# DJjjjhao/FIRA-ICSE

Measured on NVIDIA H100. Metric: train_commits_per_sec, higher is better.
Workload: dtype bf16

## Files before the change

fira_icse_b200/csrc/common.cuh:

```cuda
#pragma once
#include <cuda_runtime.h>
#include <cuda_bf16.h>
#include <stdint.h>
#include <stdio.h>

#define FIRA_OK 0
#define FIRA_ERR_SHAPE 1
#define FIRA_ERR_ALIGN 2
#define FIRA_ERR_CUDA 3
#define FIRA_ERR_DTYPE 4
#define FIRA_ERR_ARG 5

#define FIRA_F32 0
#define FIRA_BF16 1

void fira_set_error(int code, const char* fmt, ...);

#define FIRA_CHECK_ARG(cond, code, ...)                      \
  do {                                                       \
    if (!(cond)) {                                           \
      fira_set_error((code), __VA_ARGS__);                   \
      return (code);                                         \
    }                                                        \
  } while (0)

#define FIRA_CHECK_LAUNCH(name)                                                   \
  do {                                                                            \
    cudaError_t e__ = cudaGetLastError();                                         \
    if (e__ != cudaSuccess) {                                                     \
      fira_set_error(FIRA_ERR_CUDA, "%s: %s", (name), cudaGetErrorString(e__));   \
      return FIRA_ERR_CUDA;                                                       \
    }                                                                             \
  } while (0)

extern "C" int fira_num_sms(void);

static inline bool fira_aligned16(const void* p) { return (reinterpret_cast<uintptr_t>(p) & 15u) == 0; }

int fira_pdl_on();

#ifdef __CUDACC__

__device__ __forceinline__ void pdl_wait() { asm volatile("griddepcontrol.wait;" ::: "memory"); }
__device__ __forceinline__ void pdl_trigger() { asm volatile("griddepcontrol.launch_dependents;" ::: "memory"); }

template <typename... KArgs, typename... Args>
inline cudaError_t launch_k(void (*kernel)(KArgs...), dim3 grid, dim3 block, size_t smem, cudaStream_t st, Args&&... args) {
  cudaLaunchConfig_t cfg = {};
  cfg.gridDim = grid;
  cfg.blockDim = block;
  cfg.dynamicSmemBytes = smem;
  cfg.stream = st;
  cudaLaunchAttribute attr[1];
  attr[0].id = cudaLaunchAttributeProgrammaticStreamSerialization;
  attr[0].val.programmaticStreamSerializationAllowed = 1;
  cfg.attrs = attr;
  cfg.numAttrs = fira_pdl_on() ? 1 : 0;
  return cudaLaunchKernelEx(&cfg, kernel, static_cast<KArgs>(args)...);
}

constexpr int kWarp = 32;
constexpr float kLnEps = 1e-5f;
constexpr float kMaskFill = -1e9f;

__device__ __forceinline__ float warp_sum(float v) {
#pragma unroll
  for (int o = 16; o > 0; o >>= 1) v += __shfl_xor_sync(0xffffffffu, v, o);
  return v;
}
__device__ __forceinline__ float warp_max(float v) {
#pragma unroll
  for (int o = 16; o > 0; o >>= 1) v = fmaxf(v, __shfl_xor_sync(0xffffffffu, v, o));
  return v;
}

template <typename T> struct Act;
template <> struct Act<float> {
  static __device__ __forceinline__ void load8(const float* p, float* v) {
    float4 a = *reinterpret_cast<const float4*>(p);
    float4 b = *reinterpret_cast<const float4*>(p + 4);
    v[0] = a.x; v[1] = a.y; v[2] = a.z; v[3] = a.w; v[4] = b.x; v[5] = b.y; v[6] = b.z; v[7] = b.w;
  }
  static __device__ __forceinline__ void store8(float* p, const float* v) {
    *reinterpret_cast<float4*>(p) = make_float4(v[0], v[1], v[2], v[3]);
    *reinterpret_cast<float4*>(p + 4) = make_float4(v[4], v[5], v[6], v[7]);
  }
  static __device__ __forceinline__ float ld(const float* p) { return *p; }
  static __device__ __forceinline__ void st(float* p, float v) { *p = v; }
};
template <> struct Act<__nv_bfloat16> {
  static __device__ __forceinline__ void load8(const __nv_bfloat16* p, float* v) {
    uint4 r = *reinterpret_cast<const uint4*>(p);
    const __nv_bfloat162* h = reinterpret_cast<const __nv_bfloat162*>(&r);
#pragma unroll
    for (int i = 0; i < 4; ++i) { float2 f = __bfloat1622float2(h[i]); v[2 * i] = f.x; v[2 * i + 1] = f.y; }
  }
  static __device__ __forceinline__ void store8(__nv_bfloat16* p, const float* v) {
    uint4 r;
    __nv_bfloat162* h = reinterpret_cast<__nv_bfloat162*>(&r);
#pragma unroll
    for (int i = 0; i < 4; ++i) h[i] = __floats2bfloat162_rn(v[2 * i], v[2 * i + 1]);
    *reinterpret_cast<uint4*>(p) = r;
  }
  static __device__ __forceinline__ float ld(const __nv_bfloat16* p) { return __bfloat162float(*p); }
  static __device__ __forceinline__ void st(__nv_bfloat16* p, float v) { *p = __float2bfloat16_rn(v); }
};

__device__ __forceinline__ uint4 philox4(uint32_t c0, uint32_t c1, uint32_t c2, uint32_t c3,
                                         uint32_t k0, uint32_t k1) {
  const uint32_t M0 = 0xD2511F53u, M1 = 0xCD9E8D57u, W0 = 0x9E3779B9u, W1 = 0xBB67AE85u;
#pragma unroll
  for (int r = 0; r < 7; ++r) {
    uint32_t hi0 = __umulhi(M0, c0), lo0 = M0 * c0;
    uint32_t hi1 = __umulhi(M1, c2), lo1 = M1 * c2;
    uint32_t n0 = hi1 ^ c1 ^ k0, n2 = hi0 ^ c3 ^ k1;
    c0 = n0; c1 = lo1; c2 = n2; c3 = lo0;
    k0 += W0; k1 += W1;
  }
  return make_uint4(c0, c1, c2, c3);
}
__device__ __forceinline__ uint32_t dropout_keep8(uint64_t seed, uint32_t stream, uint64_t idx8, float p_drop) {
  const uint4 r = philox4((uint32_t)idx8, (uint32_t)(idx8 >> 32), stream, 0u, (uint32_t)seed, (uint32_t)(seed >> 32));
  const uint32_t thr = (uint32_t)(p_drop * 65536.0f);
  uint32_t m = 0;
  m |= ((r.x & 0xffffu) >= thr) << 0; m |= ((r.x >> 16) >= thr) << 1;
  m |= ((r.y & 0xffffu) >= thr) << 2; m |= ((r.y >> 16) >= thr) << 3;
  m |= ((r.z & 0xffffu) >= thr) << 4; m |= ((r.z >> 16) >= thr) << 5;
  m |= ((r.w & 0xffffu) >= thr) << 6; m |= ((r.w >> 16) >= thr) << 7;
  return m;
}

#endif
```

fira_icse_b200/csrc/gemm_ln.cu:

```cuda
#include <cuda.h>
#include <cudaTypedefs.h>
#include "tc_common.cuh"
#include "fira_b200.h"

namespace {

using namespace tc;

constexpr int BM = 128, BN = 256, BK = 64, STAGES = 3;
constexpr int N_CONSUMER = 256;
constexpr int THREADS = N_CONSUMER + 32;
constexpr uint32_t A_BYTES = BM * BK * 2, B_BYTES = BN * BK * 2, STAGE_BYTES = A_BYTES + B_BYTES;
constexpr uint32_t RING_BYTES = STAGES * STAGE_BYTES;
constexpr uint32_t RES_BYTES = BM * BN * 2;
constexpr uint32_t SMEM_BYTES = RING_BYTES + RES_BYTES + 1024;
constexpr uint32_t BOX = 64 * 64 * 2;
constexpr uint32_t OFF_OUT = 8 * BOX;

struct LnParams {
  int M, K;
  long split;
  const float* bias; const float* rs; const float* rc; const float* gamma; const float* beta;
  float* mean; float* rstd;
  float p_drop; uint64_t seed; const uint64_t* seed_ctr; uint32_t stream_id;
  int has_b;
};

__global__ void __launch_bounds__(THREADS, 1)
gemm_ln_kernel(const __grid_constant__ CUtensorMap tmX, const __grid_constant__ CUtensorMap tmW,
               const __grid_constant__ CUtensorMap tmR, const __grid_constant__ CUtensorMap tmZ,
               const __grid_constant__ CUtensorMap tmOA, const __grid_constant__ CUtensorMap tmOB, LnParams p) {
  extern __shared__ unsigned char smem_dyn[];
  __shared__ __align__(8) unsigned long long full_bar[STAGES], empty_bar[STAGES], res_bar;
  __shared__ __align__(16) float s_bias[BN], s_rc[BN], s_gamma[BN], s_beta[BN];
  const uint32_t base = (smem_addr(smem_dyn) + 1023u) & ~1023u;
  unsigned char* sm = smem_dyn + (base - smem_addr(smem_dyn));
  const int warp = threadIdx.x >> 5, lane = threadIdx.x & 31;
  const int m0 = blockIdx.x * BM;
  const int nkb = (p.K + BK - 1) / BK;

  if (threadIdx.x == 0) {
    for (int s = 0; s < STAGES; ++s) { mbar_init(smem_addr(&full_bar[s]), 1); mbar_init(smem_addr(&empty_bar[s]), N_CONSUMER); }
    mbar_init(smem_addr(&res_bar), 1);
    mbar_init_fence();
    tma_prefetch_desc(&tmX); tma_prefetch_desc(&tmW); tma_prefetch_desc(&tmR); tma_prefetch_desc(&tmZ);
    tma_prefetch_desc(&tmOA);
    if (p.has_b) tma_prefetch_desc(&tmOB);
  }
  __syncthreads();
  pdl_wait(); pdl_trigger();

  if (warp == N_CONSUMER / 32) {
    if (lane == 0) {
      for (int i = 0; i < nkb; ++i) {
        const int s = i % STAGES;
        mbar_wait(smem_addr(&empty_bar[s]), ((i / STAGES) & 1) ^ 1);
        const uint32_t sa = base + s * STAGE_BYTES, sb = sa + A_BYTES, fb = smem_addr(&full_bar[s]);
        mbar_expect_tx(fb, STAGE_BYTES);
        const int kb = (i + (int)blockIdx.x) % nkb;
        tma_load_2d(sa, &tmX, kb * BK, m0, fb);
        tma_load_2d(sb, &tmW, kb * BK, 0, fb);
        if (i == 0) {
          const uint32_t rb = smem_addr(&res_bar);
          mbar_expect_tx(rb, RES_BYTES);
#pragma unroll
          for (int g = 0; g < 4; ++g) tma_load_2d(base + RING_BYTES + g * 16384, &tmR, g * 64, m0, rb);
        }
      }
    }
    return;
  }

  const int wg = warp >> 2;
  for (int c = threadIdx.x; c < BN; c += N_CONSUMER) {
    s_bias[c] = p.bias ? p.bias[c] : 0.f;
    s_rc[c] = p.rs ? p.rc[c] : 0.f;
    s_gamma[c] = p.gamma[c];
    s_beta[c] = p.beta[c];
  }
  float acc[BN / 2];
#pragma unroll
  for (int i = 0; i < BN / 2; ++i) acc[i] = 0.f;
  for (int i = 0; i < nkb; ++i) {
    const int s = i % STAGES;
    mbar_wait(smem_addr(&full_bar[s]), (i / STAGES) & 1);
    const uint32_t sa = base + s * STAGE_BYTES + wg * 8192, sb = base + s * STAGE_BYTES + A_BYTES;
    wgmma_fence();
#pragma unroll
    for (int k = 0; k < BK / 16; ++k) wgmma<BN, 0, 0>(acc, make_desc(sa + k * 32, 16, 1024), make_desc(sb + k * 32, 16, 1024));
    wgmma_commit();
    wgmma_wait<1>();
    if (i > 0) mbar_arrive(smem_addr(&empty_bar[(i - 1) % STAGES]));
  }
  wgmma_wait<0>();
  reg_fence<BN / 2>(acc);
  named_bar(1, N_CONSUMER);
  mbar_wait(smem_addr(&res_bar), 0);

  const int q4 = lane & 3;
  int tr[2], br[2], m[2];
  float rsm[2];
#pragma unroll
  for (int h = 0; h < 2; ++h) {
    tr[h] = wg * 64 + (warp & 3) * 16 + (lane >> 2) + 8 * h;
    br[h] = tr[h] - wg * 64;
    m[h] = m0 + tr[h];
    rsm[h] = (p.rs && m[h] < p.M) ? p.rs[m[h]] : 0.f;
  }
  uint64_t seed = p.seed;
  if (p.seed_ctr) seed += *p.seed_ctr;
  const float keep_scale = p.p_drop > 0.f ? 1.f / (1.f - p.p_drop) : 1.f;
  const unsigned char* res = sm + RING_BYTES;
  unsigned char* zst = sm + wg * 4 * BOX;
  unsigned char* ost = sm + OFF_OUT + wg * 4 * BOX;
  const int row0 = m0 + wg * 64;
  float sum[2] = {0.f, 0.f}, sq[2] = {0.f, 0.f};
#pragma unroll
  for (int j = 0; j < BN / 8; ++j) {
    const int c = 8 * j + 2 * q4, g = j >> 3, chunk = j & 7;
    const float2 bb = *reinterpret_cast<const float2*>(s_bias + c), kk = *reinterpret_cast<const float2*>(s_rc + c);
#pragma unroll
    for (int h = 0; h < 2; ++h) {
      float v0 = fmaf(rsm[h], kk.x, acc[4 * j + 2 * h] + bb.x), v1 = fmaf(rsm[h], kk.y, acc[4 * j + 2 * h + 1] + bb.y);
      const __nv_bfloat162 zb = __floats2bfloat162_rn(v0, v1);
      *reinterpret_cast<__nv_bfloat162*>(zst + g * BOX + br[h] * 128 + ((chunk ^ (br[h] & 7)) << 4) + q4 * 4) = zb;
      const float2 zf = __bfloat1622float2(zb);
      v0 = zf.x; v1 = zf.y;
      if (p.p_drop > 0.f) {
        const uint32_t mk = dropout_keep8(seed, p.stream_id, (uint64_t)m[h] * 32 + j, p.p_drop) >> (2 * q4);
        v0 = (mk & 1) ? v0 * keep_scale : 0.f;
        v1 = (mk & 2) ? v1 * keep_scale : 0.f;
      }
      const float2 rf = __bfloat1622float2(*reinterpret_cast<const __nv_bfloat162*>(
          res + g * 16384 + tr[h] * 128 + ((chunk ^ (tr[h] & 7)) << 4) + q4 * 4));
      v0 += rf.x; v1 += rf.y;
      acc[4 * j + 2 * h] = v0; acc[4 * j + 2 * h + 1] = v1;
      sum[h] += v0 + v1;
      sq[h] = fmaf(v0, v0, fmaf(v1, v1, sq[h]));
    }
  }
  fence_proxy_async();
  named_bar(2 + wg, 128);
  if ((threadIdx.x & 127) == 0 && row0 < p.M) {
#pragma unroll
    for (int g = 0; g < 4; ++g) tma_store_2d(&tmZ, smem_addr(zst + g * BOX), g * 64, row0);
    asm volatile("cp.async.bulk.commit_group;" ::: "memory");
  }
  float mean[2], rstd[2];
#pragma unroll
  for (int h = 0; h < 2; ++h) {
    sum[h] += __shfl_xor_sync(0xffffffffu, sum[h], 1);
    sum[h] += __shfl_xor_sync(0xffffffffu, sum[h], 2);
    sq[h] += __shfl_xor_sync(0xffffffffu, sq[h], 1);
    sq[h] += __shfl_xor_sync(0xffffffffu, sq[h], 2);
    mean[h] = sum[h] * (1.f / BN);
    const float var = fmaxf(sq[h] * (1.f / BN) - mean[h] * mean[h], 0.f);
    rstd[h] = rsqrtf(var + kLnEps);
    if (q4 == 0 && m[h] < p.M) { p.mean[m[h]] = mean[h]; p.rstd[m[h]] = rstd[h]; }
  }
#pragma unroll
  for (int j = 0; j < BN / 8; ++j) {
    const int c = 8 * j + 2 * q4, g = j >> 3, chunk = j & 7;
    const float2 gg = *reinterpret_cast<const float2*>(s_gamma + c), ee = *reinterpret_cast<const float2*>(s_beta + c);
#pragma unroll
    for (int h = 0; h < 2; ++h) {
      const float o0 = fmaf((acc[4 * j + 2 * h] - mean[h]) * rstd[h], gg.x, ee.x);
      const float o1 = fmaf((acc[4 * j + 2 * h + 1] - mean[h]) * rstd[h], gg.y, ee.y);
      *reinterpret_cast<__nv_bfloat162*>(ost + g * BOX + br[h] * 128 + ((chunk ^ (br[h] & 7)) << 4) + q4 * 4) =
          __floats2bfloat162_rn(o0, o1);
    }
  }
  fence_proxy_async();
  named_bar(2 + wg, 128);
  if ((threadIdx.x & 127) == 0) {
    if (row0 < p.M) {
#pragma unroll
      for (int g = 0; g < 4; ++g) {
        if (row0 < p.split) tma_store_2d(&tmOA, smem_addr(ost + g * BOX), g * 64, row0);
#pragma unroll
        for (int hh = 0; hh < 2; ++hh)
          if (p.has_b && row0 + 32 * hh < p.M && row0 + 32 * hh + 32 > p.split)
            tma_store_2d(&tmOB, smem_addr(ost + g * BOX + hh * 4096), g * 64, row0 + 32 * hh);
      }
    }
    tma_store_commit_wait_read();
  }
}

}

extern "C" int fira_gemm_ln_fwd(const void* x, long ldx, const void* w, const float* bias, const float* rs, const float* rc,
                                const void* resid, const float* gamma, const float* beta, void* z, void* outA, void* outB,
                                long split, float* mean, float* rstd, long rows, int K, float p_drop, uint64_t seed,
                                const uint64_t* seed_ctr, uint32_t stream_id, void* stream) {
  FIRA_CHECK_ARG(x && w && resid && gamma && beta && z && outA && mean && rstd, FIRA_ERR_ARG, "gemm_ln_fwd: null argument");
  FIRA_CHECK_ARG(rows > 0 && rows < (1L << 31) && K > 0 && K % 8 == 0, FIRA_ERR_SHAPE, "gemm_ln_fwd: rows %ld K %d", rows, K);
  FIRA_CHECK_ARG(ldx % 8 == 0, FIRA_ERR_ALIGN, "gemm_ln_fwd: ldx must be a multiple of 8");
  FIRA_CHECK_ARG(fira_aligned16(x) && fira_aligned16(w) && fira_aligned16(resid) && fira_aligned16(z) && fira_aligned16(outA) &&
                     fira_aligned16(outB), FIRA_ERR_ALIGN, "gemm_ln_fwd: 16-B alignment");
  FIRA_CHECK_ARG((rs == nullptr) == (rc == nullptr), FIRA_ERR_ARG, "gemm_ln_fwd: rs/rc must come together");
  FIRA_CHECK_ARG(p_drop >= 0.f && p_drop < 1.f, FIRA_ERR_ARG, "gemm_ln_fwd: p_drop %f", p_drop);
  if (split > rows || outB == nullptr) split = rows;
  FIRA_CHECK_ARG(split >= 0, FIRA_ERR_ARG, "gemm_ln_fwd: split %ld", split);
  const int M = (int)rows;
  CUtensorMap tx, tw, tr, tz, toa, tob;
  int rc_;
  if ((rc_ = make_map_bf16(&tx, x, M, K, ldx, BK, BM, "gemm_ln_fwd"))) return rc_;
  if ((rc_ = make_map_bf16(&tw, w, BN, K, K, BK, BN, "gemm_ln_fwd"))) return rc_;
  if ((rc_ = make_map_bf16(&tr, resid, M, BN, BN, 64, BM, "gemm_ln_fwd"))) return rc_;
  if ((rc_ = make_map_bf16(&tz, z, M, BN, BN, 64, 64, "gemm_ln_fwd"))) return rc_;
  const bool has_a = split > 0, has_b = split < rows;
  if ((rc_ = make_map_bf16(&toa, outA, has_a ? split : 1, BN, BN, 64, 64, "gemm_ln_fwd"))) return rc_;
  tob = toa;
  if (has_b && (rc_ = make_map_bf16(&tob, outB, rows, BN, BN, 64, 32, "gemm_ln_fwd"))) return rc_;
  LnParams p{M, K, has_a ? split : 0, bias, rs, rc, gamma, beta, mean, rstd, p_drop, seed, seed_ctr, stream_id, has_b ? 1 : 0};
  cudaError_t e = cudaFuncSetAttribute(gemm_ln_kernel, cudaFuncAttributeMaxDynamicSharedMemorySize, (int)SMEM_BYTES);
  if (e != cudaSuccess) { fira_set_error(FIRA_ERR_CUDA, "gemm_ln attr: %s", cudaGetErrorString(e)); return FIRA_ERR_CUDA; }
  launch_k(gemm_ln_kernel, dim3((M + BM - 1) / BM), dim3(THREADS), SMEM_BYTES, (cudaStream_t)stream, tx, tw, tr, tz, toa, tob, p);
  FIRA_CHECK_LAUNCH("fira_gemm_ln_fwd");
  return FIRA_OK;
}
```

fira_icse_b200/ops.py:

```python
import os

import torch

from . import _lib
from . import optim as _optim
from ._lib import FIRA_BF16, FIRA_F32, call

D = 256

if hasattr(torch.autograd.graph, "set_warn_on_accumulate_grad_stream_mismatch"):
    torch.autograd.graph.set_warn_on_accumulate_grad_stream_mismatch(False)


def _stream():
    return torch.cuda.current_stream().cuda_stream


def _ptr(t, off=0):
    if t is None:
        return None
    return t.data_ptr() + off * t.element_size()


def _require_cuda(*ts):
    for t in ts:
        if t is not None and not t.is_cuda:
            raise _lib.FiraLibraryError(
                "fira_icse_b200: tensors must live on a CUDA device -- this package has no CPU path "
                "(the CPU reference lives in oracle/ and is test infrastructure only)")


def _ceil(a, b):
    return (a + b - 1) // b


def _gdest(ts, shape, zero=False):
    if not isinstance(ts, (list, tuple)):
        ts = (ts,)
    v = _optim.grad_dest(ts, shape)
    if v is not None:
        return v
    return (torch.zeros if zero else torch.empty)(shape, dtype=torch.float32, device=ts[0].device)


def _num_sms():
    return _lib.lib().fira_num_sms()


def _pick_splits(M, N, K, relu):
    if relu:
        return 1
    if _ceil(M, 128) * _ceil(N, 128) >= _num_sms():
        return 1
    tiles = _ceil(M, 64) * _ceil(N, 64)
    want = _ceil(2 * _num_sms(), tiles)
    return max(1, min(want, _ceil(K, 16) // 8))


def gemm_raw(A, lda, a_k, Bp, ldb, b_k, C, ldc, M, N, K, bias=None, rs=None, rc=None, relu=False,
             accumulate=False, splits=None):
    if splits is None:
        splits = _pick_splits(M, N, K, relu)
    call("fira_gemm_f32", A, lda, int(a_k), Bp, ldb, int(b_k), C, ldc, M, N, K, _ptr(bias), _ptr(rs), _ptr(rc),
         int(relu), int(accumulate), splits, _stream())


def linear(x, W, b=None, relu=False, out=None, ld_out=None, rs=None, rc=None, M=None, x_off=0, ldx=None):
    N, K = W.shape
    M = x.shape[0] if M is None else M
    ldx = K if ldx is None else ldx
    ld_out = N if ld_out is None else ld_out
    if out is None:
        out = torch.empty((M, ld_out), dtype=torch.float32, device=x.device)
    gemm_raw(_ptr(x, x_off), ldx, 1, _ptr(W), K, 1, _ptr(out), ld_out, M, N, K, bias=b, rs=rs, rc=rc, relu=relu)
    return out


def linear_dx(dy, ld_dy, W, M, out=None, accumulate=False, dy_off=0, n=None):
    N, K = W.shape
    n = N if n is None else n
    if out is None:
        out = torch.empty((M, K), dtype=torch.float32, device=dy.device)
    gemm_raw(_ptr(dy, dy_off), ld_dy, 1, _ptr(W), K, 0, _ptr(out), K, M, K, n, accumulate=accumulate)
    return out


def linear_dw(dy, ld_dy, x, ldx, M, N, K, dy_off=0, x_off=0, out=None):
    dW = torch.empty((N, K), dtype=torch.float32, device=dy.device) if out is None else out
    gemm_raw(_ptr(dy, dy_off), ld_dy, 0, _ptr(x, x_off), ldx, 0, _ptr(dW), K, N, K, M)
    return dW


def gemm_tc(A, lda, a_kmajor, Bm, ldb, b_kmajor, C, ldc, M, N, K, bias=None, rs=None, rc=None, relu=False,
            accumulate=False, splits=1, a_off=0, b_off=0, c_off=0):
    call("fira_gemm_bf16_tc", _ptr(A, a_off), lda, int(a_kmajor), _ptr(Bm, b_off), ldb, int(b_kmajor), _ptr(C, c_off),
         ldc, int(C.dtype == torch.bfloat16), M, N, K, _ptr(bias), _ptr(rs), _ptr(rc), int(relu), int(accumulate),
         splits, _stream())
    return C


_WGRAD_CTAS_ENV = os.environ.get("FIRA_WGRAD_CTAS")


def _wgrad_ctas():
    return max(1, int(_WGRAD_CTAS_ENV)) if _WGRAD_CTAS_ENV else _num_sms()


def _tc_splits(tiles, kblocks):
    wgrad_ctas = _wgrad_ctas()
    if tiles >= wgrad_ctas:
        return 1
    return max(1, min(kblocks // 8 if kblocks >= 16 else 1, _ceil(wgrad_ctas, tiles)))


def colsum(x, ld, M, N, weight=None, x_off=0, dtype=None, out=None):
    if dtype is None:
        dtype = FIRA_BF16 if x.dtype == torch.bfloat16 else FIRA_F32
    if out is None:
        out = torch.zeros(N, dtype=torch.float32, device=x.device)
    call("fira_colsum", _ptr(x, x_off), ld, M, N, _ptr(weight), _ptr(out), dtype, _stream())
    return out


class Prec:

    def __init__(self, bf16, wcache=None, seed_ctr=None):
        self.bf16 = bool(bf16)
        self.seed_ctr = seed_ctr
        self.code = FIRA_BF16 if self.bf16 else FIRA_F32
        self.tdt = torch.bfloat16 if self.bf16 else torch.float32
        self.wcache = {} if wcache is None else wcache

    def empty(self, shape, dev):
        return torch.empty(shape, dtype=self.tdt, device=dev)

    def w(self, W):
        if not self.bf16:
            return W
        m = _optim.mirror_of(W)
        if m is not None:
            return m
        k = (W.data_ptr(), tuple(W.shape))
        if k not in self.wcache:
            self.wcache[k] = (W, W.detach().to(torch.bfloat16))
        return self.wcache[k][1]

    def linear(self, x, W, b=None, relu=False, out=None, ld_out=None, rs=None, rc=None, M=None, ldx=None, x_off=0):
        if not self.bf16:
            return linear(x, W, b, relu=relu, out=out, ld_out=ld_out, rs=rs, rc=rc, M=M, ldx=ldx, x_off=x_off)
        N, K = W.shape
        M = x.shape[0] if M is None else M
        ldx = K if ldx is None else ldx
        ld_out = N if ld_out is None else ld_out
        if out is None:
            out = torch.empty((M, ld_out), dtype=torch.bfloat16, device=x.device)
        return gemm_tc(x, ldx, 1, self.w(W), K, 1, out, ld_out, M, N, K, bias=b, rs=rs, rc=rc, relu=relu, a_off=x_off)

    def linear_dx(self, dy, ld_dy, W, M, out=None, accumulate=False, dy_off=0):
        if not self.bf16:
            return linear_dx(dy, ld_dy, W, M, out=out, accumulate=accumulate, dy_off=dy_off)
        N, K = W.shape
        if out is None:
            out = torch.empty((M, K), dtype=torch.bfloat16, device=dy.device)
        return gemm_tc(dy, ld_dy, 1, self.w(W), K, 0, out, K, M, K, N, accumulate=accumulate, a_off=dy_off)

    def linear_dx_relu(self, dy, ld_dy, W, M, h):
        N, K = W.shape
        if self.bf16 and FUSE_DX_RELU:
            out = torch.empty((M, K), dtype=torch.bfloat16, device=dy.device)
            call("fira_gemm_bf16_tc_dx_relu", _ptr(dy), ld_dy, _ptr(self.w(W)), K, _ptr(out), K, _ptr(h), M, K, N, _stream())
            return out
        out = self.linear_dx(dy, ld_dy, W, M)
        call("fira_relu_bwd", _ptr(h), _ptr(out), M * K, self.code, _stream())
        return out

    def linear_dw(self, dy, ld_dy, x, ldx, M, N, K, dy_off=0, x_off=0, out=None, dbias=None):
        if not self.bf16:
            if dbias is not None:
                colsum(dy, ld_dy, M, N, x_off=dy_off, out=dbias)
            return linear_dw(dy, ld_dy, x, ldx, M, N, K, dy_off=dy_off, x_off=x_off, out=out)
        dW = torch.empty((N, K), dtype=torch.float32, device=dy.device) if out is None else out
        bn = 256 if K > 128 else (128 if K > 64 else 64)
        splits = _tc_splits(_ceil(N, 128) * _ceil(K, bn), _ceil(M, 64))
        if dbias is not None and os.environ.get("FIRA_DBIAS_FUSED", "1") != "0":
            call("fira_gemm_bf16_tc_dbias", _ptr(dy, dy_off), ld_dy, _ptr(x, x_off), ldx, 0, _ptr(dW), K, 0, N, K, M, 0, splits,
                 _ptr(dbias), _stream())
            return dW
        if dbias is not None:
            colsum(dy, ld_dy, M, N, x_off=dy_off, out=dbias)
        return gemm_tc(dy, ld_dy, 0, x, ldx, 0, dW, K, N, K, M, splits=splits, a_off=dy_off, b_off=x_off)

    def linear_ln(self, x, W, b, resid, gamma, beta, outA, outB, split, rows, p, seed, sid, rs=None, rc=None):
        N, K = W.shape
        if self.bf16 and N == D and FUSE_GEMM_LN:
            z = torch.empty((rows, D), dtype=torch.bfloat16, device=x.device)
            stats = torch.empty((2, rows), dtype=torch.float32, device=x.device)
            call("fira_gemm_ln_fwd", _ptr(x), K, _ptr(self.w(W)), _ptr(b), _ptr(rs), _ptr(rc), _ptr(resid), _ptr(gamma),
                 _ptr(beta), _ptr(z), _ptr(outA), _ptr(outB) if outB is not outA else None, split, _ptr(stats),
                 _ptr(stats, rows), rows, K, float(p), seed, _ptr(self.seed_ctr), sid, _stream())
            return z, stats
        z = self.linear(x, W, b, rs=rs, rc=rc, M=rows)
        return z, self.ln_fwd(z, resid, gamma, beta, outA, outB, split, rows, p, seed, sid)

    def ln_fwd(self, z, resid, gamma, beta, outA, outB, split, rows, p, seed, sid):
        stats = torch.empty((2, rows), dtype=torch.float32, device=z.device)
        call("fira_ln_residual_fwd", _ptr(z), _ptr(resid), _ptr(gamma), _ptr(beta), _ptr(outA), _ptr(outB), split,
             _ptr(stats), _ptr(stats, rows), rows, D, float(p), seed, _ptr(self.seed_ctr), sid, self.code, _stream())
        return stats

    def ln_bwd(self, dA, dB, split, z, resid, stats, gamma, rows, p, seed, sid, d_resid=None, accum=False, beta=None):
        dz = torch.empty_like(z)
        if d_resid is None:
            d_resid = torch.empty_like(z)
        dgb = _gdest((gamma, beta), (2, D), zero=True) if beta is not None else \
            torch.zeros((2, D), dtype=torch.float32, device=z.device)
        call("fira_ln_residual_bwd", _ptr(dA), _ptr(dB), split, _ptr(z), _ptr(resid), _ptr(stats), _ptr(stats, rows),
             _ptr(gamma), _ptr(dz), _ptr(d_resid), int(accum), _ptr(dgb), _ptr(dgb, D), rows, D, float(p), seed,
             _ptr(self.seed_ctr), sid, self.code, _stream())
        return dz, d_resid, dgb[0], dgb[1]


_F32 = Prec(False)


def ln_fwd(z, resid, gamma, beta, outA, outB, split, rows, p, seed, sid):
    return _F32.ln_fwd(z, resid, gamma, beta, outA, outB, split, rows, p, seed, sid)


def ln_bwd(dA, dB, split, z, resid, stats, gamma, rows, p, seed, sid, d_resid=None, accum=False):
    return _F32.ln_bwd(dA, dB, split, z, resid, stats, gamma, rows, p, seed, sid, d_resid=d_resid, accum=accum)


_SIDE_STREAMS = {}
N_SIDE = max(1, int(os.environ.get("FIRA_SIDE_STREAMS", "8")))
FUSE_GEMM_LN = os.environ.get("FIRA_GEMM_LN", "0") != "0"
FUSE_DX_RELU = os.environ.get("FIRA_DX_RELU", "1") != "0" and os.environ.get("FIRA_GEMM_TMA_STORE", "1") != "0"
MERGE_SPLITS = max(1, int(os.environ.get("FIRA_MERGE_SPLITS", "4")))
_TURN = [0]


class Fork:

    def __init__(self, device, n_side=None):
        self.main = torch.cuda.current_stream(device)
        key = (device.index if device.index is not None else torch.cuda.current_device())
        if key not in _SIDE_STREAMS:
            _SIDE_STREAMS[key] = [torch.cuda.Stream(device=device) for _ in range(N_SIDE)]
        self.sides = _SIDE_STREAMS[key][:n_side] if n_side else _SIDE_STREAMS[key]
        self.side = self.sides[0]
        self.keep = []
        self.used = set()

    def __call__(self, *tensors, lane=None):
        self.keep.extend(tensors)
        if lane is None:
            lane = _TURN[0]
            _TURN[0] += 1
        self.side = self.sides[lane % len(self.sides)]
        self.side.wait_stream(self.main)
        self.used.add(self.side)
        return torch.cuda.stream(self.side)

    def join(self):
        for s in self.used:
            self.main.wait_stream(s)
        self.used.clear()
        self.keep.clear()


class Prefetch:

    def __init__(self):
        self.wcache = {}
        self.items = None
        self.event = None


def _prep_encoder_layer(pr, fork, mark_emb, Wq, bq, Wk, bk, Wv, bv, Wo, W1, b1, W2, fused=True):
    f32 = dict(dtype=torch.float32, device=Wq.device)

    def done():
        ev = torch.cuda.Event()
        ev.record()
        return ev
    with fork(mark_emb, Wq, bq, Wk, bk, Wv, bv, Wo):
        Wqk = _optim.cat_rows((Wq, Wk))
        bqk = _optim.cat_rows((bq, bk))
        Vtab = linear(mark_emb, Wv, bv)
        for w in (Wqk, Wo):
            pr.w(w)
        ev_comb = done()
    with fork(W1, W2):
        Wc = torch.empty((D, D), **f32)
        gemm_raw(_ptr(W2), D, 1, _ptr(W1), D, 0, _ptr(Wc), D, D, D, D, splits=MERGE_SPLITS if pr.bf16 else 1)
        pr.w(Wc)
        WcT16 = Wc.t().contiguous().to(torch.bfloat16) if (pr.bf16 and fused) else None
        ev_wc = done()
    with fork(W2, b1):
        c1 = torch.empty((D,), **f32)
        gemm_raw(_ptr(W2), D, 1, _ptr(b1), D, 1, _ptr(c1), 1, D, 1, D, splits=1)
        ev_c1 = done()
    return (Wqk, bqk, Vtab, Wc, c1, WcT16), (ev_comb, ev_wc, ev_c1)


def prefetch_decoder(bf16, lp, device):
    pf = Prefetch()
    pr = Prec(bf16, pf.wcache)
    L = len(lp) // DEC_LAYER_PARAMS
    fork = Fork(device)
    with fork(*lp):
        Wkv = _optim.cat_rows([t for i in range(L) for t in (lp[i * 26 + 12], lp[i * 26 + 14])])
        bkv = _optim.cat_rows([t for i in range(L) for t in (lp[i * 26 + 13], lp[i * 26 + 15])])
        pr.w(Wkv)
        layers = []
        for i in range(L):
            q = lp[i * 26:(i + 1) * 26]
            Wqkv = _optim.cat_rows((q[0], q[2], q[4]))
            bqkv = _optim.cat_rows((q[1], q[3], q[5]))
            for w in (Wqkv, q[6], q[10], q[16], q[20], q[22]):
                pr.w(w)
            layers.append((Wqkv, bqkv))
        pf.items = (Wkv, bkv, layers)
        pf.event = torch.cuda.Event()
        pf.event.record()
    pf.fork = fork
    return pf


def prefetch_head(bf16, Wout, Ws, Wt):
    pf = Prefetch()
    if bf16:
        pr = Prec(True, pf.wcache)
        fork = Fork(Wout.device)
        with fork(Wout, Ws, Wt):
            for w in (Wout, Ws, Wt):
                pr.w(w)
            pf.event = torch.cuda.Event()
            pf.event.record()
        pf.fork = fork
    return pf


def make_seed():
    return int(torch.randint(0, 2 ** 62, (1,)).item())


ENC_LAYER_PARAMS = 16


class EncoderFn(torch.autograd.Function):

    @staticmethod
    def forward(ctx, cfg, sou, mark, ast_change, sub_token, edges, pos_table, emb, ast_emb, mark_emb, *lp):
        _require_cuda(sou, emb)
        B, n_code = sou.shape
        n_sub, n_ast = sub_token.shape[1], ast_change.shape[1]
        N = n_code + n_sub + n_ast
        assert edges.N == N and edges.B == B, "adjacency / batch mismatch"
        R, Mc = B * N, B * n_code
        L = len(lp) // ENC_LAYER_PARAMS
        training, seed = cfg["training"], cfg["seed"]
        p_comb = cfg["p_comb"] if training else 0.0
        p_gcn = cfg["p_gcn"] if training else 0.0
        heads = cfg["heads"]
        pr = Prec(cfg.get("bf16", False), seed_ctr=cfg.get("seed_ctr"))
        dev = emb.device
        f32 = dict(dtype=torch.float32, device=dev)
        st = _stream()

        Xc = pr.empty((Mc, D), dev)
        Gin = pr.empty((R, D), dev)
        if cfg.get("pos") is not None:
            call("fira_embed_nodes_pos_fwd", _ptr(sou), _ptr(cfg["pos"]), _ptr(sub_token), _ptr(ast_change), _ptr(emb),
                 _ptr(ast_emb), _ptr(pos_table), _ptr(Xc), _ptr(Gin), B, n_code, n_sub, n_ast, D, pr.code, st)
        else:
            call("fira_embed_nodes_fwd", _ptr(sou), _ptr(sub_token), _ptr(ast_change), _ptr(emb), _ptr(ast_emb),
                 _ptr(pos_table), _ptr(Xc), _ptr(Gin), B, n_code, n_sub, n_ast, D, pr.code, st)
        fused = pr.bf16 and os.environ.get("FIRA_GCN_FUSED", "0") != "0"
        rs = None if fused else edges.rowsum(n_code, n_sub, n_ast)
        erows = edges.rows_csr(n_code, n_sub, n_ast) if fused else None
        saved = []
        fork = Fork(dev)
        preps, events = [], []
        for i in range(L):
            Wq, bq, Wk, bk, Wv, bv, Wo, bo, clw, clb, W1, b1, W2, b2, glw, glb = lp[i * 16:(i + 1) * 16]
            t, e = _prep_encoder_layer(pr, fork, mark_emb, Wq, bq, Wk, bk, Wv, bv, Wo, W1, b1, W2, fused=fused)
            preps.append(t)
            events.append(e)
        for i in range(L):
            Wq, bq, Wk, bk, Wv, bv, Wo, bo, clw, clb, W1, b1, W2, b2, glw, glb = lp[i * 16:(i + 1) * 16]
            sid = cfg["stream_base"] + i * 8
            cur = torch.cuda.current_stream()
            cur.wait_event(events[i][0])
            Wqk, bqk, Vtab, Wc, c1, WcT16 = preps[i]
            QK = pr.linear(Xc, Wqk, bqk)
            Cd = pr.empty((Mc, D), dev)
            call("fira_comb_gate_fwd", _ptr(QK), 2 * D, _ptr(Vtab), _ptr(mark), _ptr(Cd), Mc, D, D // heads,
                 float(p_comb), seed, _ptr(pr.seed_ctr), sid + 0, pr.code, st)
            Zc, st_c = pr.linear_ln(Cd, Wo, bo, Xc, clw, clb, Gin, Gin, Mc, Mc, p_comb, seed, sid + 1)
            Xc_n = pr.empty((Mc, D), dev)
            Gin_n = pr.empty((R, D), dev)
            cur.wait_event(events[i][1])
            cur.wait_event(events[i][2])
            if fused:
                G = None
                Z = pr.empty((R, D), dev)
                st_g = torch.empty((2, R), **f32)
                call("fira_gcn_layer_fwd", _ptr(erows[0]), _ptr(erows[1]), _ptr(erows[2]), _ptr(Gin), _ptr(pr.w(Wc)),
                     _ptr(b2), _ptr(c1), _ptr(glw), _ptr(glb), _ptr(Z), _ptr(Xc_n), _ptr(Gin_n), Mc, _ptr(st_g),
                     _ptr(st_g, R), R, D, float(p_gcn), seed, _ptr(pr.seed_ctr), sid + 2, st)
            else:
                G = pr.empty((R, D), dev)
                call("fira_gcn_aggregate", _ptr(edges.rowptr), _ptr(edges.col), _ptr(edges.val), _ptr(Gin), None,
                     _ptr(G), B, n_code, n_sub, n_ast, D, pr.code, st)
                Z, st_g = pr.linear_ln(G, Wc, b2, Gin, glw, glb, Xc_n, Gin_n, Mc, R, p_gcn, seed, sid + 2, rs=rs, rc=c1)
            saved.append((Xc, QK, Vtab, Cd, Zc, st_c, Gin, G, Z, st_g, Wqk, Wc, c1, WcT16))
            Xc, Gin = Xc_n, Gin_n
        memory = pr.empty((B, n_code + n_sub, D), dev)
        call("fira_pack_memory", _ptr(Xc), _ptr(Gin), _ptr(memory), B, n_code, n_sub, D, pr.code, st)
        fork.join()

        ctx.saved = saved
        ctx.wcache = pr.wcache
        ctx.misc = (cfg, sou, mark, ast_change, sub_token, edges, rs, B, n_code, n_sub, n_ast, p_comb, p_gcn, fused)
        ctx.save_for_backward(emb, ast_emb, mark_emb, *lp)
        return memory

    @staticmethod
    def backward(ctx, d_mem):
        cfg, sou, mark, ast_change, sub_token, edges, rs, B, n_code, n_sub, n_ast, p_comb, p_gcn, fused = ctx.misc
        emb, ast_emb, mark_emb, *lp = ctx.saved_tensors
        N = n_code + n_sub + n_ast
        R, Mc = B * N, B * n_code
        L = len(lp) // ENC_LAYER_PARAMS
        seed, heads = cfg["seed"], cfg["heads"]
        pr = Prec(cfg.get("bf16", False), ctx.wcache, seed_ctr=cfg.get("seed_ctr"))
        dev = emb.device
        f32 = dict(dtype=torch.float32, device=dev)
        st = _stream()
        et = edges.t()
        etrows = et.rows_csr(n_code, n_sub, n_ast) if fused else None
        d_mem = d_mem.contiguous().to(pr.tdt)
        dXc = pr.empty((Mc, D), dev)
        dGin = pr.empty((R, D), dev)
        call("fira_unpack_memory", _ptr(d_mem), _ptr(dXc), _ptr(dGin), B, n_code, n_sub, n_ast, D, pr.code, st)
        d_mark_emb = _gdest(mark_emb, tuple(mark_emb.shape), zero=True)
        grads = [None] * len(lp)
        fork = Fork(dev)
        for i in reversed(range(L)):
            Wq, bq, Wk, bk, Wv, bv, Wo, bo, clw, clb, W1, b1, W2, b2, glw, glb = lp[i * 16:(i + 1) * 16]
            Xc, QK, Vtab, Cd, Zc, st_c, Gin, G, Z, st_g, Wqk, Wc, c1, WcT16 = ctx.saved[i]
            sid = cfg["stream_base"] + i * 8
            dZ, dRes, d_glw, d_glb = pr.ln_bwd(dXc, dGin, Mc, Z, Gin, st_g, glw, R, p_gcn, seed, sid + 2, beta=glb)
            dGin_i = pr.empty((R, D), dev)
            if fused:
                AdZ = pr.empty((R, D), dev)
                call("fira_gcn_layer_bwd", _ptr(etrows[0]), _ptr(etrows[1]), _ptr(etrows[2]), _ptr(dZ), _ptr(WcT16),
                     _ptr(dRes), _ptr(AdZ), _ptr(dGin_i), R, D, st)
            with fork(dZ, G, rs, W1, W2, b1):
                d_b2 = _gdest(b2, (D,), zero=True)
                if fused:
                    fork.keep.append(AdZ)
                    colsum(dZ, D, R, D, out=d_b2)
                    d_c1 = torch.zeros(D, dtype=torch.float32, device=dev)
                    dWc = pr.linear_dw(AdZ, D, Gin, D, R, D, D, dbias=d_c1)
                else:
                    d_c1 = colsum(dZ, D, R, D, weight=rs)
                    dWc = pr.linear_dw(dZ, D, G, D, R, D, D, dbias=d_b2)
                ev_dwc = torch.cuda.Event()
                ev_dwc.record()
                fork.keep.extend((dWc, d_c1))
            with fork():
                torch.cuda.current_stream().wait_event(ev_dwc)
                d_W2 = _gdest(W2, (D, D))
                gemm_raw(_ptr(dWc), D, 1, _ptr(W1), D, 1, _ptr(d_W2), D, D, D, D, rs=d_c1, rc=b1, splits=MERGE_SPLITS if pr.bf16 else 1)
            with fork():
                torch.cuda.current_stream().wait_event(ev_dwc)
                d_W1 = _gdest(W1, (D, D))
                gemm_raw(_ptr(W2), D, 0, _ptr(dWc), D, 0, _ptr(d_W1), D, D, D, D, splits=MERGE_SPLITS if pr.bf16 else 1)
                d_b1 = _gdest(b1, (D,))
                gemm_raw(_ptr(W2), D, 0, _ptr(d_c1), 1, 0, _ptr(d_b1), 1, D, 1, D, splits=1)
            if not fused:
                dG = pr.linear_dx(dZ, D, Wc, R)
                call("fira_gcn_aggregate", _ptr(et.rowptr), _ptr(et.col), _ptr(et.val), _ptr(dG), _ptr(dRes),
                     _ptr(dGin_i), B, n_code, n_sub, n_ast, D, pr.code, st)
            dXc_n = pr.empty((Mc, D), dev)
            dZc, _, d_clw, d_clb = pr.ln_bwd(dGin_i, dGin_i, Mc, Zc, Xc, st_c, clw, Mc, p_comb, seed, sid + 1,
                                             d_resid=dXc_n, beta=clb)
            with fork(dZc, Cd):
                d_bo = _gdest(bo, (D,), zero=True)
                d_Wo = pr.linear_dw(dZc, D, Cd, D, Mc, D, D, out=_gdest(Wo, (D, D)), dbias=d_bo)
            dCd = pr.linear_dx(dZc, D, Wo, Mc)
            dQK = pr.empty((Mc, 2 * D), dev)
            dVtab = torch.zeros((4, D), **f32)
            call("fira_comb_gate_bwd", _ptr(QK), 2 * D, _ptr(Vtab), _ptr(mark), _ptr(dCd), _ptr(dQK), _ptr(dVtab),
                 Mc, D, D // heads, float(p_comb), seed, _ptr(pr.seed_ctr), sid + 0, pr.code, st)
            with fork(dQK, Xc):
                d_bqk = _gdest((bq, bk), (2 * D,), zero=True)
                d_Wqk = pr.linear_dw(dQK, 2 * D, Xc, D, Mc, 2 * D, D, out=_gdest((Wq, Wk), (2 * D, D)), dbias=d_bqk)
            with fork(dVtab, mark_emb, Wv):
                d_Wv = linear_dw(dVtab, D, mark_emb, D, 4, D, D, out=_gdest(Wv, (D, D)))
                d_bv = colsum(dVtab, D, 4, D, out=_gdest(bv, (D,), zero=True))
            with fork(dVtab, Wv, lane=0):
                linear_dx(dVtab, D, Wv, 4, out=d_mark_emb, accumulate=True)
            pr.linear_dx(dQK, 2 * D, Wqk, Mc, out=dXc_n, accumulate=True)
            grads[i * 16:(i + 1) * 16] = [d_Wqk[:D], d_bqk[:D], d_Wqk[D:], d_bqk[D:], d_Wv, d_bv, d_Wo, d_bo,
                                          d_clw, d_clb, d_W1, d_b1, d_W2, d_b2, d_glw, d_glb]
            dXc, dGin = dXc_n, dGin_i
            ctx.saved[i] = None
        d_emb = _gdest(emb, tuple(emb.shape), zero=True)
        d_ast = _gdest(ast_emb, tuple(ast_emb.shape), zero=True)
        call("fira_embed_nodes_bwd", _ptr(sou), _ptr(sub_token), _ptr(ast_change), _ptr(dXc), _ptr(dGin),
             _ptr(d_emb), _ptr(d_ast), B, n_code, n_sub, n_ast, D, pr.code, st)
        fork.join()
        d_mark_emb[0].zero_()
        return (None, None, None, None, None, None, None, d_emb, d_ast, d_mark_emb, *grads)


DEC_LAYER_PARAMS = 26


class DecoderFn(torch.autograd.Function):

    @staticmethod
    def forward(ctx, cfg, tar, memory, mem_mask, tar_mask, pos_table, dec_emb, *lp):
        _require_cuda(tar, memory, dec_emb)
        B, T = tar.shape
        pk = cfg.get("packed")
        S = pk.S if pk is not None else memory.shape[1]
        Mt, Ms = B * T, memory.shape[0] * memory.shape[1]
        L = len(lp) // DEC_LAYER_PARAMS
        H = cfg["heads"]
        training, seed = cfg["training"], cfg["seed"]
        p = cfg["p_dec"] if training else 0.0
        pr = Prec(cfg.get("bf16", False), seed_ctr=cfg.get("seed_ctr"))
        dev = dec_emb.device
        f32 = dict(dtype=torch.float32, device=dev)
        st = _stream()
        mem_dtype = memory.dtype
        memory = memory.contiguous().to(pr.tdt)

        X = pr.empty((Mt, D), dev)
        call("fira_embed_rows_fwd", _ptr(tar), _ptr(dec_emb), _ptr(pos_table), _ptr(X), Mt, T, D, pr.code, st)
        pf = cfg.get("prefetch")
        if pf is None:
            pf = prefetch_decoder(pr.bf16, lp, dev)
        torch.cuda.current_stream().wait_event(pf.event)
        pf.fork.join()
        pr.wcache.update(pf.wcache)
        Wkv, bkv, qkv_layers = pf.items
        ldkv = L * 2 * D
        KV = pr.linear(memory.view(Ms, D), Wkv, bkv)
        saved = []
        for i in range(L):
            (sWq, sbq, sWk, sbk, sWv, sbv, sWo, sbo, slw, slb,
             cWq, cbq, cWk, cbk, cWv, cbv, cWo, cbo, clw, clb,
             fW1, fb1, fW2, fb2, flw, flb) = lp[i * 26:(i + 1) * 26]
            sid = cfg["stream_base"] + 64 + i * 8
            Wqkv, bqkv = qkv_layers[i]
            QKV = pr.linear(X, Wqkv, bqkv)
            ctx1 = pr.empty((Mt, D), dev)
            st1 = torch.empty((B, H, T, 2), **f32)
            call("fira_attn_fwd", _ptr(QKV), 3 * D, _ptr(QKV, D), 3 * D, _ptr(QKV, 2 * D), 3 * D, _ptr(tar_mask), 1,
                 _ptr(ctx1), D, _ptr(st1), B, H, T, T, D // H, pr.code, st)
            X1 = pr.empty((Mt, D), dev)
            Z1, ls1 = pr.linear_ln(ctx1, sWo, sbo, X, slw, slb, X1, X1, Mt, Mt, p, seed, sid + 0)
            Q = pr.linear(X1, cWq, cbq)
            ctx2 = pr.empty((Mt, D), dev)
            st2 = torch.empty((B, H, T, 2), **f32)
            if pk is not None:
                call("fira_attn_packed_fwd", _ptr(Q), D, _ptr(KV, i * 2 * D), ldkv, _ptr(KV, i * 2 * D + D), ldkv,
                     _ptr(pk.ranges), Ms, _ptr(mem_mask), S, pk.chunks, _ptr(ctx2), D, _ptr(st2), B, H, T, D // H, pr.code, st)
            else:
                call("fira_attn_fwd", _ptr(Q), D, _ptr(KV, i * 2 * D), ldkv, _ptr(KV, i * 2 * D + D), ldkv,
                     _ptr(mem_mask), 0, _ptr(ctx2), D, _ptr(st2), B, H, T, S, D // H, pr.code, st)
            X2 = pr.empty((Mt, D), dev)
            Z2, ls2 = pr.linear_ln(ctx2, cWo, cbo, X1, clw, clb, X2, X2, Mt, Mt, p, seed, sid + 1)
            Hh = pr.linear(X2, fW1, fb1, relu=True)
            X3 = pr.empty((Mt, D), dev)
            Z3, ls3 = pr.linear_ln(Hh, fW2, fb2, X2, flw, flb, X3, X3, Mt, Mt, p, seed, sid + 2)
            saved.append((X, Wqkv, QKV, ctx1, st1, Z1, ls1, X1, Q, ctx2, st2, Z2, ls2, X2, Hh, Z3, ls3))
            X = X3
        ctx.saved = saved
        ctx.wcache = pr.wcache
        ctx.misc = (cfg, tar, memory, mem_mask, tar_mask, KV, Wkv, B, T, S, p, mem_dtype, Ms)
        ctx.save_for_backward(dec_emb, *lp)
        return X.view(B, T, D)

    @staticmethod
    def backward(ctx, d_out):
        cfg, tar, memory, mem_mask, tar_mask, KV, Wkv, B, T, S, p, mem_dtype, Ms = ctx.misc
        dec_emb, *lp = ctx.saved_tensors
        Mt = B * T
        pk = cfg.get("packed")
        L = len(lp) // DEC_LAYER_PARAMS
        H, seed = cfg["heads"], cfg["seed"]
        pr = Prec(cfg.get("bf16", False), ctx.wcache, seed_ctr=cfg.get("seed_ctr"))
        dev = dec_emb.device
        st = _stream()
        ldkv = L * 2 * D
        dX = d_out.contiguous().to(pr.tdt).view(Mt, D)
        dKV = pr.empty((Ms, ldkv), dev)
        if pk is not None:
            call("fira_zero_pad_rows", _ptr(dKV), ldkv, ldkv, _ptr(pk.off), B, pk.Rc, pk.Rs, pr.code, st)
        grads = [None] * len(lp)
        F = 4 * D
        fork = Fork(dev)
        for i in reversed(range(L)):
            (sWq, sbq, sWk, sbk, sWv, sbv, sWo, sbo, slw, slb,
             cWq, cbq, cWk, cbk, cWv, cbv, cWo, cbo, clw, clb,
             fW1, fb1, fW2, fb2, flw, flb) = lp[i * 26:(i + 1) * 26]
            X, Wqkv, QKV, ctx1, st1, Z1, ls1, X1, Q, ctx2, st2, Z2, ls2, X2, Hh, Z3, ls3 = ctx.saved[i]
            sid = cfg["stream_base"] + 64 + i * 8
            dZ3, dX2, d_flw, d_flb = pr.ln_bwd(dX, dX, Mt, Z3, X2, ls3, flw, Mt, p, seed, sid + 2, beta=flb)
            with fork(dZ3, Hh):
                d_fb2 = _gdest(fb2, (D,), zero=True)
                d_fW2 = pr.linear_dw(dZ3, D, Hh, F, Mt, D, F, out=_gdest(fW2, (D, F)), dbias=d_fb2)
            dHh = pr.linear_dx_relu(dZ3, D, fW2, Mt, Hh)
            with fork(dHh, X2):
                d_fb1 = _gdest(fb1, (F,), zero=True)
                d_fW1 = pr.linear_dw(dHh, F, X2, D, Mt, F, D, out=_gdest(fW1, (F, D)), dbias=d_fb1)
            pr.linear_dx(dHh, F, fW1, Mt, out=dX2, accumulate=True)
            dZ2, dX1, d_clw, d_clb = pr.ln_bwd(dX2, dX2, Mt, Z2, X1, ls2, clw, Mt, p, seed, sid + 1, beta=clb)
            with fork(dZ2, ctx2):
                d_cbo = _gdest(cbo, (D,), zero=True)
                d_cWo = pr.linear_dw(dZ2, D, ctx2, D, Mt, D, D, out=_gdest(cWo, (D, D)), dbias=d_cbo)
            dctx2 = pr.linear_dx(dZ2, D, cWo, Mt)
            dQ = pr.empty((Mt, D), dev)
            if pk is not None:
                call("fira_attn_packed_bwd", _ptr(Q), D, _ptr(KV, i * 2 * D), ldkv, _ptr(KV, i * 2 * D + D), ldkv,
                     _ptr(pk.ranges), Ms, _ptr(mem_mask), S, pk.chunks, _ptr(ctx2), _ptr(dctx2), D, _ptr(st2), _ptr(dQ), D,
                     _ptr(dKV, i * 2 * D), ldkv, _ptr(dKV, i * 2 * D + D), ldkv, B, H, T, D // H, pr.code, st)
            else:
                call("fira_attn_bwd", _ptr(Q), D, _ptr(KV, i * 2 * D), ldkv, _ptr(KV, i * 2 * D + D), ldkv,
                     _ptr(mem_mask), 0, _ptr(ctx2), _ptr(dctx2), D, _ptr(st2), _ptr(dQ), D, _ptr(dKV, i * 2 * D), ldkv,
                     _ptr(dKV, i * 2 * D + D), ldkv, B, H, T, S, D // H, pr.code, st)
            with fork(dQ, X1):
                d_cbq = _gdest(cbq, (D,), zero=True)
                d_cWq = pr.linear_dw(dQ, D, X1, D, Mt, D, D, out=_gdest(cWq, (D, D)), dbias=d_cbq)
            pr.linear_dx(dQ, D, cWq, Mt, out=dX1, accumulate=True)
            dZ1, dX0, d_slw, d_slb = pr.ln_bwd(dX1, dX1, Mt, Z1, X, ls1, slw, Mt, p, seed, sid + 0, beta=slb)
            with fork(dZ1, ctx1):
                d_sbo = _gdest(sbo, (D,), zero=True)
                d_sWo = pr.linear_dw(dZ1, D, ctx1, D, Mt, D, D, out=_gdest(sWo, (D, D)), dbias=d_sbo)
            dctx1 = pr.linear_dx(dZ1, D, sWo, Mt)
            dQKV = pr.empty((Mt, 3 * D), dev)
            call("fira_attn_bwd", _ptr(QKV), 3 * D, _ptr(QKV, D), 3 * D, _ptr(QKV, 2 * D), 3 * D, _ptr(tar_mask), 1,
                 _ptr(ctx1), _ptr(dctx1), D, _ptr(st1), _ptr(dQKV), 3 * D, _ptr(dQKV, D), 3 * D, _ptr(dQKV, 2 * D), 3 * D,
                 B, H, T, T, D // H, pr.code, st)
            with fork(dQKV, X):
                d_bqkv = _gdest((sbq, sbk, sbv), (3 * D,), zero=True)
                d_Wqkv = pr.linear_dw(dQKV, 3 * D, X, D, Mt, 3 * D, D, out=_gdest((sWq, sWk, sWv), (3 * D, D)), dbias=d_bqkv)
            pr.linear_dx(dQKV, 3 * D, Wqkv, Mt, out=dX0, accumulate=True)
            grads[i * 26:(i + 1) * 26] = [
                d_Wqkv[:D], d_bqkv[:D], d_Wqkv[D:2 * D], d_bqkv[D:2 * D], d_Wqkv[2 * D:], d_bqkv[2 * D:],
                d_sWo, d_sbo, d_slw, d_slb,
                d_cWq, d_cbq, None, None, None, None, d_cWo, d_cbo, d_clw, d_clb,
                d_fW1, d_fb1, d_fW2, d_fb2, d_flw, d_flb]
            dX = dX0
            ctx.saved[i] = None
        mem2 = memory.view(Ms, D)
        with fork(dKV, mem2):
            kv_w = [t for i in range(L) for t in (lp[i * 26 + 12], lp[i * 26 + 14])]
            kv_b = [t for i in range(L) for t in (lp[i * 26 + 13], lp[i * 26 + 15])]
            d_bkv = _gdest(kv_b, (ldkv,), zero=True)
            d_Wkv = pr.linear_dw(dKV, ldkv, mem2, D, Ms, ldkv, D, out=_gdest(kv_w, (ldkv, D)), dbias=d_bkv)
        d_mem = pr.linear_dx(dKV, ldkv, Wkv, Ms).view(memory.shape).to(mem_dtype)
        for i in range(L):
            o = i * 2 * D
            grads[i * 26 + 12], grads[i * 26 + 13] = d_Wkv[o:o + D], d_bkv[o:o + D]
            grads[i * 26 + 14], grads[i * 26 + 15] = d_Wkv[o + D:o + 2 * D], d_bkv[o + D:o + 2 * D]
        d_emb = _gdest(dec_emb, tuple(dec_emb.shape), zero=True)
        call("fira_embed_rows_bwd", _ptr(tar), _ptr(dX), _ptr(d_emb), Mt, D, pr.code, st)
        fork.join()
        return (None, None, d_mem, None, None, None, d_emb, *grads)


def _ld_logits(V):
    return (V + 63) // 64 * 64


def copy_scores_fwd(pr, memory2, dec2, Ws, Wt, wres, bres, B, T, S, src_mask=None, row_mask=None, ranges=None):
    src = pr.linear(memory2, Ws)
    tgt = pr.linear(dec2, Wt)
    sc = torch.empty((B, T, S), dtype=torch.float32, device=dec2.device)
    if ranges is not None:
        call("fira_copy_scores_packed_fwd", _ptr(src), _ptr(tgt), _ptr(wres), _ptr(bres), _ptr(ranges), _ptr(src_mask),
             _ptr(row_mask), _ptr(sc), B, T, S, D, pr.code, _stream())
    else:
        call("fira_copy_scores_fwd", _ptr(src), _ptr(tgt), _ptr(wres), _ptr(bres), _ptr(src_mask), _ptr(row_mask),
             _ptr(sc), B, T, S, D, pr.code, _stream())
    return src, tgt, sc


class HeadFn(torch.autograd.Function):

    @staticmethod
    def forward(ctx, want_argmax, bf16, pf, memory, dec, mem_mask, label, Wout, bout, Ws, Wt, Wres, bres, Wp, bp,
                pk=None):
        _require_cuda(memory, dec, Wout)
        B, T = dec.shape[0], dec.shape[1]
        S = pk.S if pk is not None else memory.shape[1]
        V = Wout.shape[0]
        Mt, Ms = B * T, memory.shape[0] * memory.shape[1]
        pr = Prec(bf16)
        if pf is not None and pf.event is not None:
            torch.cuda.current_stream().wait_event(pf.event)
            pf.fork.join()
            pr.wcache.update(pf.wcache)
        dev = dec.device
        f32 = dict(dtype=torch.float32, device=dev)
        st = _stream()
        memory2 = memory.contiguous().to(pr.tdt).view(Ms, D)
        dec2 = dec.contiguous().to(pr.tdt).view(Mt, D)
        dec32 = dec2 if not pr.bf16 else dec2.float()
        ldl = _ld_logits(V)
        logits = pr.empty((Mt, ldl), dev)
        pr.linear(dec2, Wout, bout, out=logits, ld_out=ldl)
        row_mask = None if want_argmax else (label >= V).to(torch.uint8)
        src, tgt, sc = copy_scores_fwd(pr, memory2, dec2, Ws, Wt, Wres, bres, B, T, S, src_mask=mem_mask,
                                       row_mask=row_mask, ranges=pk.ranges if pk is not None else None)
        gl = linear(dec32, Wp, bp)
        stats = torch.empty((Mt, 8), **f32)
        nll = torch.empty((Mt,), **f32)
        amax = torch.empty((Mt,), dtype=torch.int32, device=dev) if want_argmax else None
        call("fira_pointer_mix_nll_fwd", _ptr(logits), ldl, _ptr(sc), _ptr(gl), _ptr(mem_mask), _ptr(label),
             _ptr(stats), _ptr(nll), _ptr(amax), Mt, T, V, S, pr.code, st)
        ctx.misc = (pr, memory2, dec2, dec32, mem_mask, label, logits, ldl, src, tgt, sc, stats, B, T, S, V,
                    memory.dtype, dec.dtype, pk, memory.shape)
        ctx.save_for_backward(Wout, Ws, Wt, Wres, Wp, bout, bres, bp)
        loss_sum = colsum(nll, 1, Mt, 1).view(())
        ids = amax.view(B, T) if want_argmax else None
        nll2 = nll.view(B, T)
        ctx.mark_non_differentiable(*([nll2, ids] if ids is not None else [nll2]))
        return loss_sum, nll2, ids

    @staticmethod
    def backward(ctx, g_loss, g_nll, g_ids):
        (pr, memory2, dec2, dec32, mem_mask, label, logits, ldl, src, tgt, sc, stats, B, T, S, V,
         mem_dt, dec_dt, pk, mem_shape) = ctx.misc
        Wout, Ws, Wt, Wres, Wp, bout, bres, bp = ctx.saved_tensors
        Mt, Ms = B * T, memory2.shape[0]
        dev = dec2.device
        f32 = dict(dtype=torch.float32, device=dev)
        st = _stream()
        up = g_loss.contiguous().float()
        dlogits = pr.empty((Mt, ldl), dev)
        dsc = torch.empty((B, T, S), **f32)
        dgl = torch.empty((Mt, 2), **f32)
        active = torch.empty((Mt,), dtype=torch.uint8, device=dev)
        call("fira_pointer_mix_nll_bwd", _ptr(logits), ldl, _ptr(sc), _ptr(mem_mask), _ptr(label), _ptr(stats),
             _ptr(up), _ptr(dlogits), _ptr(dsc), _ptr(dgl), _ptr(active), Mt, T, V, S, pr.code, st)
        d_src = pr.empty((Ms, D), dev)
        d_tgt = torch.zeros((Mt, D), **f32)
        d_wres = _gdest(Wres, (1, D), zero=True)
        d_bres = _gdest(bres, (1,), zero=True)
        if pk is not None:
            call("fira_zero_pad_rows", _ptr(d_src), D, D, _ptr(pk.off), B, pk.Rc, pk.Rs, pr.code, st)
            call("fira_copy_scores_packed_bwd", _ptr(src), _ptr(tgt), _ptr(Wres), _ptr(dsc), _ptr(active), _ptr(pk.ranges),
                 _ptr(d_src), _ptr(d_tgt), _ptr(d_wres), _ptr(d_bres), B, T, S, D, pr.code, st)
        else:
            call("fira_copy_scores_bwd", _ptr(src), _ptr(tgt), _ptr(Wres), _ptr(dsc), _ptr(active), _ptr(d_src),
                 _ptr(d_tgt), _ptr(d_wres), _ptr(d_bres), B, T, S, D, pr.code, st)
        fork = Fork(dev)
        with fork(d_src, memory2):
            d_Ws = pr.linear_dw(d_src, D, memory2, D, Ms, D, D, out=_gdest(Ws, (D, D)))
        with fork(dlogits, dec2):
            d_bout = _gdest(bout, (V,), zero=True)
            d_Wout = pr.linear_dw(dlogits, ldl, dec2, D, Mt, V, D, out=_gdest(Wout, (V, D)), dbias=d_bout)
        with fork(dgl, dec32, d_tgt):
            d_bp = colsum(dgl, 2, Mt, 2, out=_gdest(bp, (2,), zero=True))
            d_Wp = linear_dw(dgl, 2, dec32, D, Mt, 2, D, out=_gdest(Wp, (2, D)))
            d_Wt = linear_dw(d_tgt, D, dec32, D, Mt, D, D, out=_gdest(Wt, (D, D)))
        d_mem = pr.linear_dx(d_src, D, Ws, Ms)
        if pr.bf16:
            d_dec = torch.empty((Mt, D), **f32)
            gemm_tc(dlogits, ldl, 1, pr.w(Wout), D, 0, d_dec, D, Mt, D, V,
                    splits=_tc_splits(_ceil(Mt, 128), _ceil(V, 64)))
        else:
            d_dec = linear_dx(dlogits, ldl, Wout, Mt)
        linear_dx(dgl, 2, Wp, Mt, out=d_dec, accumulate=True)
        linear_dx(d_tgt, D, Wt, Mt, out=d_dec, accumulate=True)
        fork.join()
        return (None, None, None, d_mem.view(mem_shape).to(mem_dt), d_dec.view(B, T, D).to(dec_dt), None, None, d_Wout,
                d_bout, d_Ws, d_Wt, d_wres, d_bres, d_Wp, d_bp, None)


class LinearFn(torch.autograd.Function):

    @staticmethod
    def forward(ctx, x, W, b):
        _require_cuda(x, W)
        N, K = W.shape
        x2 = x.contiguous().float().view(-1, K)
        M = x2.shape[0]
        ld = (N + 3) // 4 * 4
        out = torch.empty((M, ld), dtype=torch.float32, device=x.device)
        linear(x2, W, b, out=out, ld_out=ld)
        ctx.save_for_backward(x2, W)
        ctx.has_bias = b is not None
        ctx.shape = x.shape
        return out[:, :N].view(*x.shape[:-1], N)

    @staticmethod
    def backward(ctx, dy):
        x2, W = ctx.saved_tensors
        N, K = W.shape
        M = x2.shape[0]
        dy2 = dy.contiguous().float().view(M, N)
        dx = linear_dx(dy2, N, W, M).view(ctx.shape)
        dW = linear_dw(dy2, N, x2, K, M, N, K)
        db = colsum(dy2, N, M, N) if ctx.has_bias else None
        return dx, dW, db


class CopyScoresFn(torch.autograd.Function):

    @staticmethod
    def forward(ctx, memory, dec, Ws, Wt, Wres, bres):
        _require_cuda(memory, dec, Ws)
        B, S, _ = memory.shape
        T = dec.shape[1]
        memory2 = memory.contiguous().float().view(B * S, D)
        dec2 = dec.contiguous().float().view(B * T, D)
        src, tgt, sc = copy_scores_fwd(_F32, memory2, dec2, Ws, Wt, Wres, bres, B, T, S)
        ctx.misc = (memory2, dec2, src, tgt, B, T, S)
        ctx.save_for_backward(Ws, Wt, Wres)
        return sc

    @staticmethod
    def backward(ctx, dsc):
        memory2, dec2, src, tgt, B, T, S = ctx.misc
        Ws, Wt, Wres = ctx.saved_tensors
        Mt, Ms = B * T, B * S
        f32 = dict(dtype=torch.float32, device=dec2.device)
        dsc = dsc.contiguous().float()
        active = torch.ones((Mt,), dtype=torch.uint8, device=dec2.device)
        d_src = torch.empty((Ms, D), **f32)
        d_tgt = torch.zeros((Mt, D), **f32)
        d_wres = torch.zeros((1, D), **f32)
        d_bres = torch.zeros((1,), **f32)
        call("fira_copy_scores_bwd", _ptr(src), _ptr(tgt), _ptr(Wres), _ptr(dsc), _ptr(active), _ptr(d_src),
             _ptr(d_tgt), _ptr(d_wres), _ptr(d_bres), B, T, S, D, FIRA_F32, _stream())
        d_Ws = linear_dw(d_src, D, memory2, D, Ms, D, D)
        d_mem = linear_dx(d_src, D, Ws, Ms).view(B, S, D)
        d_Wt = linear_dw(d_tgt, D, dec2, D, Mt, D, D)
        d_dec = linear_dx(d_tgt, D, Wt, Mt).view(B, T, D)
        return d_mem, d_dec, d_Ws, d_Wt, d_wres, d_bres
```

include/fira_b200.h:

```cpp
#ifndef FIRA_B200_H_
#define FIRA_B200_H_

#include <stdint.h>

#ifdef __cplusplus
extern "C" {
#endif

#define FIRA_F32 0
#define FIRA_BF16 1
#define FIRA_EDGE_F32 0
#define FIRA_EDGE_BF16 1
#define FIRA_EDGE_F64 2

int fira_version(void);
const char* fira_last_error_string(void);
int fira_built_arch(void);
int fira_num_sms(void);
int fira_set_pdl(int on);
int fira_get_pdl(void);

int fira_gemm_f32(const float* A, long lda, int a_kcontig, const float* B, long ldb, int b_kcontig, float* C,
                  long ldc, int M, int N, int K, const float* bias, const float* rs, const float* rc, int relu,
                  int accumulate, int splits, void* stream);

int fira_gemm_bf16_tc(const void* A, long lda, int a_kmajor, const void* B, long ldb, int b_kmajor, void* C,
                      long ldc, int c_is_bf16, int M, int N, int K, const float* bias, const float* rs,
                      const float* rc, int relu, int accumulate, int splits, void* stream);

int fira_gemm_bf16_tc_dbias(const void* A, long lda, const void* B, long ldb, int b_kmajor, void* C, long ldc,
                            int c_is_bf16, int M, int N, int K, int accumulate, int splits, float* d_bias, void* stream);

int fira_gemm_ln_fwd(const void* x, long ldx, const void* w, const float* bias, const float* rs, const float* rc,
                     const void* resid, const float* gamma, const float* beta, void* z, void* outA, void* outB, long split,
                     float* mean, float* rstd, long rows, int K, float p_drop, uint64_t seed, const uint64_t* seed_ctr,
                     uint32_t stream_id, void* stream);

int fira_gemm_bf16_tc_dx_relu(const void* dy, long lddy, const void* W, long ldw, void* dx, long lddx, const void* h,
                              int M, int N, int K, void* stream);

int fira_debug_set_probe(void* probe);

int fira_embed_nodes_fwd(const int* sou, const int* sub_token, const int* ast_change, const float* emb,
                         const float* ast_emb, const float* pos_table, void* out_code, void* out_rest, int B,
                         int n_code, int n_sub, int n_ast, int dim, int dtype, void* stream);
int fira_embed_nodes_pos_fwd(const int* sou, const int* pos, const int* sub_token, const int* ast_change,
                             const float* emb, const float* ast_emb, const float* pos_table, void* out_code,
                             void* out_rest, int B, int n_code, int n_sub, int n_ast, int dim, int dtype, void* stream);
int fira_zero_pad_rows(void* x, long ld, int width, const int* off, int B, int Rc, int Rs, int dtype, void* stream);
int fira_embed_nodes_bwd(const int* sou, const int* sub_token, const int* ast_change, const void* d_code,
                         const void* d_rest, float* d_emb, float* d_ast_emb, int B, int n_code, int n_sub, int n_ast,
                         int dim, int dtype, void* stream);
int fira_embed_rows_fwd(const int* ids, const float* emb, const float* pos_table, void* out, long rows, int period,
                        int dim, int dtype, void* stream);
int fira_embed_rows_bwd(const int* ids, const void* d_out, float* d_emb, long rows, int dim, int dtype, void* stream);

int fira_ln_residual_fwd(const void* z, const void* resid, const float* gamma, const float* beta, void* outA,
                         void* outB, long split, float* mean, float* rstd, long rows, int dim, float p_drop,
                         uint64_t seed, const uint64_t* seed_ctr, uint32_t stream_id, int dtype, void* stream);
int fira_ln_residual_bwd(const void* d_outA, const void* d_outB, long split, const void* z, const void* resid,
                         const float* mean, const float* rstd, const float* gamma, void* d_z, void* d_resid,
                         int d_resid_accum, float* d_gamma, float* d_beta, long rows, int dim, float p_drop,
                         uint64_t seed, const uint64_t* seed_ctr, uint32_t stream_id, int dtype, void* stream);

int fira_comb_gate_fwd(const void* qk, long ld_qk, const float* vtab, const int* mark, void* out, long rows, int dim,
                       int d_head, float p_drop, uint64_t seed, const uint64_t* seed_ctr, uint32_t stream_id, int dtype, void* stream);
int fira_comb_gate_bwd(const void* qk, long ld_qk, const float* vtab, const int* mark, const void* d_out, void* d_qk,
                       float* d_vtab, long rows, int dim, int d_head, float p_drop, uint64_t seed, const uint64_t* seed_ctr,
                       uint32_t stream_id, int dtype, void* stream);

int fira_comb_gate3_fwd(const void* q, const void* k, const void* v, void* out, long rows, int dim, int d_head,
                        float p_drop, uint64_t seed, const uint64_t* seed_ctr, uint32_t stream_id, int dtype, void* stream);
int fira_comb_gate3_bwd(const void* q, const void* k, const void* v, const void* d_out, void* d_q, void* d_k, void* d_v,
                        long rows, int dim, int d_head, float p_drop, uint64_t seed, const uint64_t* seed_ctr,
                        uint32_t stream_id, int dtype, void* stream);

int fira_relu_bwd(const void* h, void* d, long n, int dtype, void* stream);
int fira_colsum(const void* x, long ld, long M, int N, const float* row_weight, float* out, int dtype, void* stream);

int fira_adam_flat(float* p, const float* g, float* m, float* v, void* p_bf16, long n, float lr, float beta1, float beta2,
                   float eps, const float* step, const float* grad_scale, void* stream);
int fira_cast_bf16(const float* x, void* y, long n, void* stream);

int fira_pack_memory(const void* code, const void* rest, void* mem, int B, int n_code, int n_sub, int dim, int dtype,
                     void* stream);
int fira_unpack_memory(const void* d_mem, void* d_code, void* d_rest, int B, int n_code, int n_sub, int n_ast, int dim,
                       int dtype, void* stream);

int fira_csr_count_dense(const void* edge, int edge_dtype, long stride_b, long stride_i, long stride_j, int B, int N,
                         int* counts, int* rowptr, void* stream);
int fira_csr_fill_dense(const void* edge, int edge_dtype, long stride_b, long stride_i, long stride_j, int B, int N,
                        const int* rowptr, int* col, float* val, void* stream);
int fira_csr_rowsum(const int* rowptr, const float* val, int B, int n_code, int n_sub, int n_ast, float* out,
                    void* stream);
int fira_gcn_aggregate(const int* rowptr, const int* col, const float* val, const void* x, const void* addend,
                       void* y, int B, int n_code, int n_sub, int n_ast, int dim, int dtype, void* stream);

int fira_csr_to_rows(const int* rowptr, const int* col, const float* val, int B, int n_code, int n_sub, int n_ast,
                     int* counts, int* rowptr_rows, int* col_rows, float* val_rows, void* stream);
int fira_gcn_layer_fwd(const int* rowptr_rows, const int* col_rows, const float* val_rows, const void* h,
                       const void* w_merged, const float* bias, const float* c1, const float* gamma, const float* beta,
                       void* z, void* outA, void* outB, long split, float* mean, float* rstd, long rows, int dim,
                       float p_drop, uint64_t seed, const uint64_t* seed_ctr, uint32_t stream_id, void* stream);
int fira_gcn_layer_bwd(const int* rowptr_rows_t, const int* col_rows_t, const float* val_rows_t, const void* d_z,
                       const void* w_merged_t, const void* d_resid, void* agg_dz, void* d_h, long rows, int dim,
                       void* stream);

int fira_attn_fwd(const void* q, long ldq, const void* k, long ldk, const void* v, long ldv,
                  const unsigned char* key_mask, int causal, void* ctx, long ldo, float* stats, int B, int H, int Lq,
                  int Lk, int d_head, int dtype, void* stream);
int fira_attn_bwd(const void* q, long ldq, const void* k, long ldk, const void* v, long ldv,
                  const unsigned char* key_mask, int causal, const void* ctx, const void* d_ctx, long ldo,
                  const float* stats, void* dq, long lddq, void* dk, long lddk, void* dv, long lddv, int B, int H,
                  int Lq, int Lk, int d_head, int dtype, void* stream);

int fira_attn_packed_fwd(const void* q, long ldq, const void* k, long ldk, const void* v, long ldv, const int* ranges,
                         long kv_rows, const unsigned char* key_mask, int mask_pitch, int max_chunks, void* ctx, long ldo,
                         float* stats, int B, int H, int Lq, int d_head, int dtype, void* stream);
int fira_attn_packed_bwd(const void* q, long ldq, const void* k, long ldk, const void* v, long ldv, const int* ranges,
                         long kv_rows, const unsigned char* key_mask, int mask_pitch, int max_chunks, const void* ctx,
                         const void* d_ctx, long ldo, const float* stats, void* dq, long lddq, void* dk, long lddk,
                         void* dv, long lddv, int B, int H, int Lq, int d_head, int dtype, void* stream);

int fira_copy_scores_fwd(const void* src_proj, const void* tgt_proj, const float* w_res, const float* b_res,
                         const unsigned char* src_mask, const unsigned char* row_mask, float* scores,
                         int B, int T_len, int S, int dim, int dtype, void* stream);
int fira_copy_scores_bwd(const void* src_proj, const void* tgt_proj, const float* w_res, const float* d_scores,
                         const unsigned char* row_active, void* d_src_proj, float* d_tgt_proj, float* d_w_res,
                         float* d_b_res, int B, int T_len, int S, int dim, int dtype, void* stream);

int fira_copy_scores_packed_fwd(const void* src_proj, const void* tgt_proj, const float* w_res, const float* b_res,
                                const int* ranges, const unsigned char* src_mask, const unsigned char* row_mask,
                                float* scores, int B, int T_len, int S, int dim, int dtype, void* stream);
int fira_copy_scores_packed_bwd(const void* src_proj, const void* tgt_proj, const float* w_res, const float* d_scores,
                                const unsigned char* row_active, const int* ranges, void* d_src_proj, float* d_tgt_proj,
                                float* d_w_res, float* d_b_res, int B, int T_len, int S, int dim, int dtype, void* stream);

int fira_pointer_mix_nll_fwd(const void* logits, long ld_logits, const float* copy_scores, const float* gate_logits,
                             const unsigned char* mem_mask, const int* label, float* stats, float* nll,
                             int* argmax_out, long rows, int T_len, int V, int S, int dtype, void* stream);
int fira_pointer_mix_nll_bwd(const void* logits, long ld_logits, const float* copy_scores,
                             const unsigned char* mem_mask, const int* label, const float* stats,
                             const float* upstream, void* d_logits, float* d_copy_scores, float* d_gate_logits,
                             unsigned char* row_active, long rows, int T_len, int V, int S, int dtype, void* stream);

int fira_pointer_mix_sample(const void* logits, long ld_logits, const float* copy_scores, const float* gate_logits,
                            const unsigned char* mem_mask, const int* copy_src, const uint64_t* seed,
                            const int* first_index, const float* uniforms, float temperature, int top_k, float top_p,
                            int eos_id, int pad_id, int* next_tok, int* seq, int* raw, float* token_logprob,
                            unsigned char* tok_mask, long ld_out, int pos, unsigned char* finished, int* length,
                            float* logprob, int B, int N, int V, int S, int dtype, void* stream);

int fira_host_build_adjacency(const int* change_code, int n_change_code, const int* change_ast, int n_change_ast,
                              const int* ast_code, int n_ast_code, const int* ast_ast, int n_ast_ast,
                              const int* code_sub, int n_code_sub, int n_diff, int n_ast, int diff_len, int sub_len,
                              int ast_change_len, int* deg, int* col, double* val, int cap, int* nnz_out);
int fira_host_batch_dims(const int* sou, const int* sub_token, const int* ast_change, const long* index, int batch,
                         int diff_len, int sub_len, int ast_change_len, int mult_code, int mult_sub, int mult_ast,
                         int* dims);
int fira_host_gather_batch(const int* sou, const int* tar, const int* mark, const int* ast_change,
                           const int* tar_label, const int* sub_token, const unsigned char* deg, const short* col,
                           const double* val, const long* edge_ptr, const long* index, int batch, int diff_len,
                           int sub_len, int ast_change_len, int msg_len, int vocab_size, const int* dims,
                           long* o_sou, long* o_tar, long* o_mark, long* o_ast_change, long* o_tar_label,
                           long* o_sub_token, int* o_rowptr, int* o_col, float* o_val, long edge_cap, int* nnz_out);

int fira_host_packed_dims(const int* sou, const int* sub_token, const int* ast_change, const unsigned char* deg,
                          const long* index, int batch, int diff_len, int sub_len, int ast_change_len, int* dims);
int fira_host_gather_packed(const int* sou, const int* tar, const int* mark, const int* ast_change,
                            const int* tar_label, const int* sub_token, const unsigned char* deg, const short* col,
                            const double* val, const long* edge_ptr, const long* index, int batch, int diff_len,
                            int sub_len, int ast_change_len, int msg_len, int vocab_size, const int* pad_dims,
                            int* o_code, int* o_mark, int* o_pos, int* o_sub, int* o_ast, int* o_off, int* o_ranges,
                            unsigned char* o_mem_mask, int* o_tar, int* o_label, unsigned char* o_tar_mask,
                            int* o_rowptr, int* o_col, float* o_val, long edge_cap, int* nnz_out);

#ifdef __cplusplus
}
#endif
#endif
```

Measured before the change: 18080.

## Split GEMM+LayerNorm across 4-CTA clusters and fuse dx GEMM into LN backward

```diff
diff --git a/fira_icse_b200/csrc/common.cuh b/fira_icse_b200/csrc/common.cuh
--- a/fira_icse_b200/csrc/common.cuh
+++ b/fira_icse_b200/csrc/common.cuh
@@ -45,18 +45,33 @@
 __device__ __forceinline__ void pdl_trigger() { asm volatile("griddepcontrol.launch_dependents;" ::: "memory"); }
 
 template <typename... KArgs, typename... Args>
-inline cudaError_t launch_k(void (*kernel)(KArgs...), dim3 grid, dim3 block, size_t smem, cudaStream_t st, Args&&... args) {
+inline cudaError_t launch_k_cluster(void (*kernel)(KArgs...), dim3 grid, dim3 block, size_t smem, cudaStream_t st,
+                                    unsigned cluster_x, Args&&... args) {
   cudaLaunchConfig_t cfg = {};
   cfg.gridDim = grid;
   cfg.blockDim = block;
   cfg.dynamicSmemBytes = smem;
   cfg.stream = st;
-  cudaLaunchAttribute attr[1];
-  attr[0].id = cudaLaunchAttributeProgrammaticStreamSerialization;
-  attr[0].val.programmaticStreamSerializationAllowed = 1;
+  cudaLaunchAttribute attr[2];
+  unsigned n = 0;
+  if (fira_pdl_on()) {
+    attr[n].id = cudaLaunchAttributeProgrammaticStreamSerialization;
+    attr[n++].val.programmaticStreamSerializationAllowed = 1;
+  }
+  if (cluster_x > 1) {
+    attr[n].id = cudaLaunchAttributeClusterDimension;
+    attr[n].val.clusterDim.x = cluster_x;
+    attr[n].val.clusterDim.y = 1;
+    attr[n++].val.clusterDim.z = 1;
+  }
   cfg.attrs = attr;
-  cfg.numAttrs = fira_pdl_on() ? 1 : 0;
+  cfg.numAttrs = n;
   return cudaLaunchKernelEx(&cfg, kernel, static_cast<KArgs>(args)...);
+}
+
+template <typename... KArgs, typename... Args>
+inline cudaError_t launch_k(void (*kernel)(KArgs...), dim3 grid, dim3 block, size_t smem, cudaStream_t st, Args&&... args) {
+  return launch_k_cluster(kernel, grid, block, smem, st, 1u, static_cast<Args&&>(args)...);
 }
 
 constexpr int kWarp = 32;
diff --git a/fira_icse_b200/csrc/gemm_ln.cu b/fira_icse_b200/csrc/gemm_ln.cu
--- a/fira_icse_b200/csrc/gemm_ln.cu
+++ b/fira_icse_b200/csrc/gemm_ln.cu
@@ -7,17 +7,118 @@
 
 using namespace tc;
 
-constexpr int BM = 128, BN = 256, BK = 64, STAGES = 3;
-constexpr int N_CONSUMER = 256;
-constexpr int THREADS = N_CONSUMER + 32;
-constexpr uint32_t A_BYTES = BM * BK * 2, B_BYTES = BN * BK * 2, STAGE_BYTES = A_BYTES + B_BYTES;
-constexpr uint32_t RING_BYTES = STAGES * STAGE_BYTES;
-constexpr uint32_t RES_BYTES = BM * BN * 2;
-constexpr uint32_t SMEM_BYTES = RING_BYTES + RES_BYTES + 1024;
-constexpr uint32_t BOX = 64 * 64 * 2;
-constexpr uint32_t OFF_OUT = 8 * BOX;
-
-struct LnParams {
+constexpr int BN = 64, BK = 64, STAGES = 4;
+constexpr int CLUSTER = 4;
+constexpr uint32_t B_BYTES = BN * BK * 2;
+
+template <int WG>
+struct Cfg {
+  static constexpr int BM = 64 * WG;
+  static constexpr int N_CONSUMER = 128 * WG;
+  static constexpr int THREADS = N_CONSUMER + 32;
+  static constexpr uint32_t A_BYTES = BM * BK * 2;
+  static constexpr uint32_t STAGE_BYTES = A_BYTES + B_BYTES;
+  static constexpr uint32_t RING_BYTES = STAGES * STAGE_BYTES;
+  static constexpr uint32_t TILE_BYTES = BM * BN * 2;
+  static constexpr uint32_t smem(int tiles) { return RING_BYTES + tiles * TILE_BYTES + 1024; }
+};
+
+__device__ __forceinline__ uint32_t cluster_rank() {
+  uint32_t r;
+  asm volatile("mov.u32 %0, %%cluster_ctarank;" : "=r"(r));
+  return r;
+}
+__device__ __forceinline__ void cluster_sync() {
+  asm volatile("barrier.cluster.arrive.release.aligned;\n\tbarrier.cluster.wait.acquire.aligned;" ::: "memory");
+}
+__device__ __forceinline__ uint32_t mapa(uint32_t a, uint32_t rank) {
+  uint32_t r;
+  asm volatile("mapa.shared::cluster.u32 %0, %1, %2;" : "=r"(r) : "r"(a), "r"(rank));
+  return r;
+}
+__device__ __forceinline__ void st_async(uint32_t a, float v, uint32_t bar) {
+  asm volatile("st.async.shared::cluster.mbarrier::complete_tx::bytes.b32 [%0], %1, [%2];"
+               ::"r"(a), "r"(__float_as_uint(v)), "r"(bar) : "memory");
+}
+__device__ __forceinline__ void st_async2(uint32_t a, float v0, float v1, uint32_t bar) {
+  asm volatile("st.async.shared::cluster.mbarrier::complete_tx::bytes.v2.b32 [%0], {%1, %2}, [%3];"
+               ::"r"(a), "r"(__float_as_uint(v0)), "r"(__float_as_uint(v1)), "r"(bar) : "memory");
+}
+
+__device__ __forceinline__ uint32_t frag_off(int r, int j, int q4) { return r * 128 + ((j ^ (r & 7)) << 4) + q4 * 4; }
+
+__device__ __forceinline__ uint32_t keep_bits(uint64_t seed, uint32_t stream_id, int m, int n0, float p_drop, int lane) {
+  const int q4 = lane & 3;
+  const uint32_t a = dropout_keep8(seed, stream_id, (uint64_t)m * 32 + n0 / 8 + q4, p_drop);
+  const uint32_t b = dropout_keep8(seed, stream_id, (uint64_t)m * 32 + n0 / 8 + q4 + 4, p_drop);
+  uint32_t bits = 0;
+#pragma unroll
+  for (int j = 0; j < BN / 8; ++j) {
+    const uint32_t mk = __shfl_sync(0xffffffffu, j < 4 ? a : b, (lane & ~3) | (j & 3));
+    bits |= ((mk >> (2 * q4)) & 3u) << (2 * j);
+  }
+  return bits;
+}
+
+template <int WG, int TB>
+__device__ __forceinline__ void produce(const CUtensorMap* tmA, const CUtensorMap* tmB, const CUtensorMap* const* tiles,
+                                        int ntiles, uint32_t tiles_dst, uint32_t tiles_bar, uint32_t base,
+                                        unsigned long long* full_bar, unsigned long long* empty_bar, int m0, int n0,
+                                        int nkb, int rank) {
+  using C = Cfg<WG>;
+  mbar_expect_tx(tiles_bar, ntiles * C::TILE_BYTES);
+  for (int t = 0; t < ntiles; ++t) tma_load_2d(tiles_dst + t * C::TILE_BYTES, tiles[t], n0, m0, tiles_bar);
+  for (int i = 0; i < nkb; ++i) {
+    const int s = i % STAGES;
+    mbar_wait(smem_addr(&empty_bar[s]), ((i / STAGES) & 1) ^ 1);
+    const uint32_t sa = base + s * C::STAGE_BYTES, sb = sa + C::A_BYTES, fb = smem_addr(&full_bar[s]);
+    mbar_expect_tx(fb, C::STAGE_BYTES);
+    const int k0 = ((i + rank) % nkb) * BK;
+    tma_load_2d(sa, tmA, k0, m0, fb);
+    if (TB) tma_load_2d(sb, tmB, n0, k0, fb);
+    else tma_load_2d(sb, tmB, k0, n0, fb);
+  }
+}
+
+template <int WG, int TB>
+__device__ __forceinline__ void consume(float* acc, int nkb, uint32_t base, unsigned long long* full_bar,
+                                        unsigned long long* empty_bar, int wg) {
+  using C = Cfg<WG>;
+#pragma unroll
+  for (int i = 0; i < BN / 2; ++i) acc[i] = 0.f;
+  for (int i = 0; i < nkb; ++i) {
+    const int s = i % STAGES;
+    mbar_wait(smem_addr(&full_bar[s]), (i / STAGES) & 1);
+    const uint32_t sa = base + s * C::STAGE_BYTES + wg * 8192, sb = base + s * C::STAGE_BYTES + C::A_BYTES;
+    wgmma_fence();
+#pragma unroll
+    for (int k = 0; k < BK / 16; ++k)
+      wgmma<BN, 0, TB>(acc, make_desc(sa + k * 32, 16, 1024), TB ? make_desc(sb + k * 2048, 8192, 1024) : make_desc(sb + k * 32, 16, 1024));
+    wgmma_commit();
+    wgmma_wait<1>();
+    if (i > 0) mbar_arrive(smem_addr(&empty_bar[(i - 1) % STAGES]));
+  }
+  wgmma_wait<0>();
+  reg_fence<BN / 2>(acc);
+}
+
+template <int WG>
+__device__ __forceinline__ void init_barriers(unsigned long long* full_bar, unsigned long long* empty_bar,
+                                              unsigned long long* tiles_bar, unsigned long long* red_bar, int rounds,
+                                              uint32_t bytes_per_round) {
+  if (threadIdx.x == 0) {
+    for (int s = 0; s < STAGES; ++s) { mbar_init(smem_addr(&full_bar[s]), 1); mbar_init(smem_addr(&empty_bar[s]), Cfg<WG>::N_CONSUMER); }
+    mbar_init(smem_addr(tiles_bar), 1);
+    for (int r = 0; r < rounds; ++r) {
+      mbar_init(smem_addr(&red_bar[r]), 1);
+      mbar_expect_tx(smem_addr(&red_bar[r]), bytes_per_round);
+    }
+    mbar_init_fence();
+  }
+  cluster_sync();
+}
+
+struct FwdParams {
   int M, K;
   long split;
   const float* bias; const float* rs; const float* rc; const float* gamma; const float* beta;
@@ -26,165 +127,352 @@
   int has_b;
 };
 
-__global__ void __launch_bounds__(THREADS, 1)
-gemm_ln_kernel(const __grid_constant__ CUtensorMap tmX, const __grid_constant__ CUtensorMap tmW,
-               const __grid_constant__ CUtensorMap tmR, const __grid_constant__ CUtensorMap tmZ,
-               const __grid_constant__ CUtensorMap tmOA, const __grid_constant__ CUtensorMap tmOB, LnParams p) {
+template <int WG>
+__global__ void __launch_bounds__(Cfg<WG>::THREADS, 1)
+gemm_ln_fwd_kernel(const __grid_constant__ CUtensorMap tmX, const __grid_constant__ CUtensorMap tmW,
+                   const __grid_constant__ CUtensorMap tmR, const __grid_constant__ CUtensorMap tmZ,
+                   const __grid_constant__ CUtensorMap tmOA, const __grid_constant__ CUtensorMap tmOB, FwdParams p) {
+  using C = Cfg<WG>;
+  constexpr int BM = C::BM;
   extern __shared__ unsigned char smem_dyn[];
-  __shared__ __align__(8) unsigned long long full_bar[STAGES], empty_bar[STAGES], res_bar;
-  __shared__ __align__(16) float s_bias[BN], s_rc[BN], s_gamma[BN], s_beta[BN];
+  __shared__ __align__(8) unsigned long long full_bar[STAGES], empty_bar[STAGES], tiles_bar, red_bar[2];
+  __shared__ __align__(16) float red[2][CLUSTER][BM];
   const uint32_t base = (smem_addr(smem_dyn) + 1023u) & ~1023u;
   unsigned char* sm = smem_dyn + (base - smem_addr(smem_dyn));
   const int warp = threadIdx.x >> 5, lane = threadIdx.x & 31;
-  const int m0 = blockIdx.x * BM;
+  const int rank = (int)cluster_rank();
+  const int m0 = blockIdx.y * BM, n0 = rank * BN;
   const int nkb = (p.K + BK - 1) / BK;
-
+  unsigned char* res = sm + C::RING_BYTES;
+  unsigned char* zst = res + C::TILE_BYTES;
+
+  init_barriers<WG>(full_bar, empty_bar, &tiles_bar, red_bar, 2, CLUSTER * BM * 4);
   if (threadIdx.x == 0) {
-    for (int s = 0; s < STAGES; ++s) { mbar_init(smem_addr(&full_bar[s]), 1); mbar_init(smem_addr(&empty_bar[s]), N_CONSUMER); }
-    mbar_init(smem_addr(&res_bar), 1);
-    mbar_init_fence();
     tma_prefetch_desc(&tmX); tma_prefetch_desc(&tmW); tma_prefetch_desc(&tmR); tma_prefetch_desc(&tmZ);
     tma_prefetch_desc(&tmOA);
     if (p.has_b) tma_prefetch_desc(&tmOB);
   }
-  __syncthreads();
   pdl_wait(); pdl_trigger();
 
-  if (warp == N_CONSUMER / 32) {
+  if (warp == C::N_CONSUMER / 32) {
     if (lane == 0) {
-      for (int i = 0; i < nkb; ++i) {
-        const int s = i % STAGES;
-        mbar_wait(smem_addr(&empty_bar[s]), ((i / STAGES) & 1) ^ 1);
-        const uint32_t sa = base + s * STAGE_BYTES, sb = sa + A_BYTES, fb = smem_addr(&full_bar[s]);
-        mbar_expect_tx(fb, STAGE_BYTES);
-        const int kb = (i + (int)blockIdx.x) % nkb;
-        tma_load_2d(sa, &tmX, kb * BK, m0, fb);
-        tma_load_2d(sb, &tmW, kb * BK, 0, fb);
-        if (i == 0) {
-          const uint32_t rb = smem_addr(&res_bar);
-          mbar_expect_tx(rb, RES_BYTES);
-#pragma unroll
-          for (int g = 0; g < 4; ++g) tma_load_2d(base + RING_BYTES + g * 16384, &tmR, g * 64, m0, rb);
-        }
-      }
+      const CUtensorMap* tiles[1] = {&tmR};
+      produce<WG, 0>(&tmX, &tmW, tiles, 1, smem_addr(res), smem_addr(&tiles_bar), base, full_bar, empty_bar, m0, n0, nkb, rank);
     }
     return;
   }
 
-  const int wg = warp >> 2;
-  for (int c = threadIdx.x; c < BN; c += N_CONSUMER) {
-    s_bias[c] = p.bias ? p.bias[c] : 0.f;
-    s_rc[c] = p.rs ? p.rc[c] : 0.f;
-    s_gamma[c] = p.gamma[c];
-    s_beta[c] = p.beta[c];
-  }
-  float acc[BN / 2];
-#pragma unroll
-  for (int i = 0; i < BN / 2; ++i) acc[i] = 0.f;
-  for (int i = 0; i < nkb; ++i) {
-    const int s = i % STAGES;
-    mbar_wait(smem_addr(&full_bar[s]), (i / STAGES) & 1);
-    const uint32_t sa = base + s * STAGE_BYTES + wg * 8192, sb = base + s * STAGE_BYTES + A_BYTES;
-    wgmma_fence();
-#pragma unroll
-    for (int k = 0; k < BK / 16; ++k) wgmma<BN, 0, 0>(acc, make_desc(sa + k * 32, 16, 1024), make_desc(sb + k * 32, 16, 1024));
-    wgmma_commit();
-    wgmma_wait<1>();
-    if (i > 0) mbar_arrive(smem_addr(&empty_bar[(i - 1) % STAGES]));
-  }
-  wgmma_wait<0>();
-  reg_fence<BN / 2>(acc);
-  named_bar(1, N_CONSUMER);
-  mbar_wait(smem_addr(&res_bar), 0);
-
-  const int q4 = lane & 3;
-  int tr[2], br[2], m[2];
+  const int wg = warp >> 2, q4 = lane & 3;
+  int tr[2], m[2];
   float rsm[2];
 #pragma unroll
   for (int h = 0; h < 2; ++h) {
     tr[h] = wg * 64 + (warp & 3) * 16 + (lane >> 2) + 8 * h;
-    br[h] = tr[h] - wg * 64;
     m[h] = m0 + tr[h];
     rsm[h] = (p.rs && m[h] < p.M) ? p.rs[m[h]] : 0.f;
   }
   uint64_t seed = p.seed;
   if (p.seed_ctr) seed += *p.seed_ctr;
   const float keep_scale = p.p_drop > 0.f ? 1.f / (1.f - p.p_drop) : 1.f;
-  const unsigned char* res = sm + RING_BYTES;
-  unsigned char* zst = sm + wg * 4 * BOX;
-  unsigned char* ost = sm + OFF_OUT + wg * 4 * BOX;
+  float bias[BN / 4], rc[BN / 4], gam[BN / 4], bet[BN / 4];
+#pragma unroll
+  for (int j = 0; j < BN / 8; ++j)
+#pragma unroll
+    for (int e = 0; e < 2; ++e) {
+      const int n = n0 + 8 * j + 2 * q4 + e;
+      bias[2 * j + e] = p.bias ? p.bias[n] : 0.f;
+      rc[2 * j + e] = p.rs ? p.rc[n] : 0.f;
+      gam[2 * j + e] = p.gamma[n];
+      bet[2 * j + e] = p.beta[n];
+    }
+  uint32_t keep[2] = {0xffffffffu, 0xffffffffu};
+  if (p.p_drop > 0.f)
+#pragma unroll
+    for (int h = 0; h < 2; ++h) keep[h] = keep_bits(seed, p.stream_id, m[h], n0, p.p_drop, lane);
   const int row0 = m0 + wg * 64;
-  float sum[2] = {0.f, 0.f}, sq[2] = {0.f, 0.f};
+
+  float acc[BN / 2];
+  consume<WG, 0>(acc, nkb, base, full_bar, empty_bar, wg);
+  mbar_wait(smem_addr(&tiles_bar), 0);
+
+  float sum[2] = {0.f, 0.f};
 #pragma unroll
   for (int j = 0; j < BN / 8; ++j) {
-    const int c = 8 * j + 2 * q4, g = j >> 3, chunk = j & 7;
-    const float2 bb = *reinterpret_cast<const float2*>(s_bias + c), kk = *reinterpret_cast<const float2*>(s_rc + c);
 #pragma unroll
     for (int h = 0; h < 2; ++h) {
-      float v0 = fmaf(rsm[h], kk.x, acc[4 * j + 2 * h] + bb.x), v1 = fmaf(rsm[h], kk.y, acc[4 * j + 2 * h + 1] + bb.y);
+      float v0 = fmaf(rsm[h], rc[2 * j], acc[4 * j + 2 * h] + bias[2 * j]);
+      float v1 = fmaf(rsm[h], rc[2 * j + 1], acc[4 * j + 2 * h + 1] + bias[2 * j + 1]);
       const __nv_bfloat162 zb = __floats2bfloat162_rn(v0, v1);
-      *reinterpret_cast<__nv_bfloat162*>(zst + g * BOX + br[h] * 128 + ((chunk ^ (br[h] & 7)) << 4) + q4 * 4) = zb;
+      *reinterpret_cast<__nv_bfloat162*>(zst + frag_off(tr[h], j, q4)) = zb;
       const float2 zf = __bfloat1622float2(zb);
       v0 = zf.x; v1 = zf.y;
       if (p.p_drop > 0.f) {
-        const uint32_t mk = dropout_keep8(seed, p.stream_id, (uint64_t)m[h] * 32 + j, p.p_drop) >> (2 * q4);
+        const uint32_t mk = keep[h] >> (2 * j);
         v0 = (mk & 1) ? v0 * keep_scale : 0.f;
         v1 = (mk & 2) ? v1 * keep_scale : 0.f;
       }
-      const float2 rf = __bfloat1622float2(*reinterpret_cast<const __nv_bfloat162*>(
-          res + g * 16384 + tr[h] * 128 + ((chunk ^ (tr[h] & 7)) << 4) + q4 * 4));
+      const float2 rf = __bfloat1622float2(*reinterpret_cast<const __nv_bfloat162*>(res + frag_off(tr[h], j, q4)));
       v0 += rf.x; v1 += rf.y;
       acc[4 * j + 2 * h] = v0; acc[4 * j + 2 * h + 1] = v1;
       sum[h] += v0 + v1;
-      sq[h] = fmaf(v0, v0, fmaf(v1, v1, sq[h]));
     }
   }
   fence_proxy_async();
   named_bar(2 + wg, 128);
   if ((threadIdx.x & 127) == 0 && row0 < p.M) {
-#pragma unroll
-    for (int g = 0; g < 4; ++g) tma_store_2d(&tmZ, smem_addr(zst + g * BOX), g * 64, row0);
+    tma_store_2d(&tmZ, smem_addr(zst + wg * 8192), n0, row0);
     asm volatile("cp.async.bulk.commit_group;" ::: "memory");
   }
-  float mean[2], rstd[2];
+
+  auto exchange = [&](int round, float* v, float* total) {
+#pragma unroll
+    for (int h = 0; h < 2; ++h) {
+      v[h] += __shfl_xor_sync(0xffffffffu, v[h], 1);
+      v[h] += __shfl_xor_sync(0xffffffffu, v[h], 2);
+      st_async(mapa(smem_addr(&red[round][rank][tr[h]]), q4), v[h], mapa(smem_addr(&red_bar[round]), q4));
+    }
+    mbar_wait(smem_addr(&red_bar[round]), 0);
+#pragma unroll
+    for (int h = 0; h < 2; ++h) total[h] = ((red[round][0][tr[h]] + red[round][1][tr[h]]) + red[round][2][tr[h]]) + red[round][3][tr[h]];
+  };
+  float mean[2], rstd[2], tot[2];
+  exchange(0, sum, tot);
+  float sq[2] = {0.f, 0.f};
 #pragma unroll
   for (int h = 0; h < 2; ++h) {
-    sum[h] += __shfl_xor_sync(0xffffffffu, sum[h], 1);
-    sum[h] += __shfl_xor_sync(0xffffffffu, sum[h], 2);
-    sq[h] += __shfl_xor_sync(0xffffffffu, sq[h], 1);
-    sq[h] += __shfl_xor_sync(0xffffffffu, sq[h], 2);
-    mean[h] = sum[h] * (1.f / BN);
-    const float var = fmaxf(sq[h] * (1.f / BN) - mean[h] * mean[h], 0.f);
-    rstd[h] = rsqrtf(var + kLnEps);
-    if (q4 == 0 && m[h] < p.M) { p.mean[m[h]] = mean[h]; p.rstd[m[h]] = rstd[h]; }
-  }
+    mean[h] = tot[h] * (1.f / (CLUSTER * BN));
+#pragma unroll
+    for (int j = 0; j < BN / 8; ++j) {
+      const float d0 = acc[4 * j + 2 * h] - mean[h], d1 = acc[4 * j + 2 * h + 1] - mean[h];
+      sq[h] = fmaf(d0, d0, fmaf(d1, d1, sq[h]));
+    }
+  }
+  exchange(1, sq, tot);
+#pragma unroll
+  for (int h = 0; h < 2; ++h) {
+    rstd[h] = rsqrtf(tot[h] * (1.f / (CLUSTER * BN)) + kLnEps);
+    if (rank == 0 && q4 == 0 && m[h] < p.M) { p.mean[m[h]] = mean[h]; p.rstd[m[h]] = rstd[h]; }
+  }
+
 #pragma unroll
   for (int j = 0; j < BN / 8; ++j) {
-    const int c = 8 * j + 2 * q4, g = j >> 3, chunk = j & 7;
-    const float2 gg = *reinterpret_cast<const float2*>(s_gamma + c), ee = *reinterpret_cast<const float2*>(s_beta + c);
 #pragma unroll
     for (int h = 0; h < 2; ++h) {
-      const float o0 = fmaf((acc[4 * j + 2 * h] - mean[h]) * rstd[h], gg.x, ee.x);
-      const float o1 = fmaf((acc[4 * j + 2 * h + 1] - mean[h]) * rstd[h], gg.y, ee.y);
-      *reinterpret_cast<__nv_bfloat162*>(ost + g * BOX + br[h] * 128 + ((chunk ^ (br[h] & 7)) << 4) + q4 * 4) =
-          __floats2bfloat162_rn(o0, o1);
+      const float o0 = fmaf((acc[4 * j + 2 * h] - mean[h]) * rstd[h], gam[2 * j], bet[2 * j]);
+      const float o1 = fmaf((acc[4 * j + 2 * h + 1] - mean[h]) * rstd[h], gam[2 * j + 1], bet[2 * j + 1]);
+      *reinterpret_cast<__nv_bfloat162*>(res + frag_off(tr[h], j, q4)) = __floats2bfloat162_rn(o0, o1);
     }
   }
   fence_proxy_async();
   named_bar(2 + wg, 128);
   if ((threadIdx.x & 127) == 0) {
     if (row0 < p.M) {
-#pragma unroll
-      for (int g = 0; g < 4; ++g) {
-        if (row0 < p.split) tma_store_2d(&tmOA, smem_addr(ost + g * BOX), g * 64, row0);
-#pragma unroll
-        for (int hh = 0; hh < 2; ++hh)
-          if (p.has_b && row0 + 32 * hh < p.M && row0 + 32 * hh + 32 > p.split)
-            tma_store_2d(&tmOB, smem_addr(ost + g * BOX + hh * 4096), g * 64, row0 + 32 * hh);
+      const uint32_t ost = smem_addr(res + wg * 8192);
+      if (row0 < p.split) tma_store_2d(&tmOA, ost, n0, row0);
+#pragma unroll
+      for (int hh = 0; hh < 2; ++hh)
+        if (p.has_b && row0 + 32 * hh < p.M && row0 + 32 * hh + 32 > p.split)
+          tma_store_2d(&tmOB, ost + hh * 4096, n0, row0 + 32 * hh);
+    }
+    tma_store_commit_wait_read();
+  }
+}
+
+struct BwdParams {
+  int M, K;
+  const float* mean; const float* rstd; const float* gamma;
+  float* d_gamma; float* d_beta;
+  float p_drop; uint64_t seed; const uint64_t* seed_ctr; uint32_t stream_id;
+};
+
+template <int WG>
+__global__ void __launch_bounds__(Cfg<WG>::THREADS, 1)
+gemm_dx_ln_bwd_kernel(const __grid_constant__ CUtensorMap tmDY, const __grid_constant__ CUtensorMap tmW,
+                      const __grid_constant__ CUtensorMap tmZ, const __grid_constant__ CUtensorMap tmR,
+                      const __grid_constant__ CUtensorMap tmAdd, const __grid_constant__ CUtensorMap tmDZ,
+                      const __grid_constant__ CUtensorMap tmDR, BwdParams p) {
+  using C = Cfg<WG>;
+  constexpr int BM = C::BM;
+  extern __shared__ unsigned char smem_dyn[];
+  __shared__ __align__(8) unsigned long long full_bar[STAGES], empty_bar[STAGES], tiles_bar, red_bar[1];
+  __shared__ __align__(16) float2 red[CLUSTER][BM];
+  __shared__ __align__(16) float colred[2][WG * 4][BN];
+  const uint32_t base = (smem_addr(smem_dyn) + 1023u) & ~1023u;
+  unsigned char* sm = smem_dyn + (base - smem_addr(smem_dyn));
+  const int warp = threadIdx.x >> 5, lane = threadIdx.x & 31;
+  const int rank = (int)cluster_rank();
+  const int m0 = blockIdx.y * BM, n0 = rank * BN;
+  const int nkb = (p.K + BK - 1) / BK;
+  unsigned char* zt = sm + C::RING_BYTES;
+  unsigned char* rt = zt + C::TILE_BYTES;
+  unsigned char* at = rt + C::TILE_BYTES;
+
+  init_barriers<WG>(full_bar, empty_bar, &tiles_bar, red_bar, 1, CLUSTER * BM * 8);
+  if (threadIdx.x == 0) {
+    tma_prefetch_desc(&tmDY); tma_prefetch_desc(&tmW); tma_prefetch_desc(&tmZ); tma_prefetch_desc(&tmR);
+    tma_prefetch_desc(&tmAdd); tma_prefetch_desc(&tmDZ); tma_prefetch_desc(&tmDR);
+  }
+  pdl_wait(); pdl_trigger();
+
+  if (warp == C::N_CONSUMER / 32) {
+    if (lane == 0) {
+      const CUtensorMap* tiles[3] = {&tmZ, &tmR, &tmAdd};
+      produce<WG, 1>(&tmDY, &tmW, tiles, 3, smem_addr(zt), smem_addr(&tiles_bar), base, full_bar, empty_bar, m0, n0, nkb, rank);
+    }
+    return;
+  }
+
+  const int wg = warp >> 2, q4 = lane & 3;
+  int tr[2], m[2];
+  float mean[2], rstd[2];
+#pragma unroll
+  for (int h = 0; h < 2; ++h) {
+    tr[h] = wg * 64 + (warp & 3) * 16 + (lane >> 2) + 8 * h;
+    m[h] = m0 + tr[h];
+    mean[h] = m[h] < p.M ? p.mean[m[h]] : 0.f;
+    rstd[h] = m[h] < p.M ? p.rstd[m[h]] : 0.f;
+  }
+  uint64_t seed = p.seed;
+  if (p.seed_ctr) seed += *p.seed_ctr;
+  const float keep_scale = p.p_drop > 0.f ? 1.f / (1.f - p.p_drop) : 1.f;
+  float gam[BN / 4];
+#pragma unroll
+  for (int j = 0; j < BN / 8; ++j) {
+    gam[2 * j] = p.gamma[n0 + 8 * j + 2 * q4];
+    gam[2 * j + 1] = p.gamma[n0 + 8 * j + 2 * q4 + 1];
+  }
+  uint32_t keep[2] = {0xffffffffu, 0xffffffffu};
+  if (p.p_drop > 0.f)
+#pragma unroll
+    for (int h = 0; h < 2; ++h) keep[h] = keep_bits(seed, p.stream_id, m[h], n0, p.p_drop, lane);
+  const int row0 = m0 + wg * 64;
+
+  float acc[BN / 2];
+  consume<WG, 1>(acc, nkb, base, full_bar, empty_bar, wg);
+  mbar_wait(smem_addr(&tiles_bar), 0);
+
+  float dxh[BN / 2], dg[BN / 4], db[BN / 4], s1[2] = {0.f, 0.f}, s2[2] = {0.f, 0.f};
+#pragma unroll
+  for (int j = 0; j < BN / 8; ++j) {
+    dg[2 * j] = dg[2 * j + 1] = db[2 * j] = db[2 * j + 1] = 0.f;
+#pragma unroll
+    for (int h = 0; h < 2; ++h) {
+      const uint32_t o = frag_off(tr[h], j, q4);
+      const float2 ad = __bfloat1622float2(*reinterpret_cast<const __nv_bfloat162*>(at + o));
+      const float2 g = __bfloat1622float2(__floats2bfloat162_rn(acc[4 * j + 2 * h] + ad.x, acc[4 * j + 2 * h + 1] + ad.y));
+      float2 y = __bfloat1622float2(*reinterpret_cast<const __nv_bfloat162*>(zt + o));
+      const float2 x = __bfloat1622float2(*reinterpret_cast<const __nv_bfloat162*>(rt + o));
+      if (p.p_drop > 0.f) {
+        const uint32_t mk = keep[h] >> (2 * j);
+        y.x = (mk & 1) ? y.x * keep_scale : 0.f;
+        y.y = (mk & 2) ? y.y * keep_scale : 0.f;
       }
-    }
-    tma_store_commit_wait_read();
-  }
+      const float xh0 = (y.x + x.x - mean[h]) * rstd[h], xh1 = (y.y + x.y - mean[h]) * rstd[h];
+      const float d0 = g.x * gam[2 * j], d1 = g.y * gam[2 * j + 1];
+      dg[2 * j] += g.x * xh0; dg[2 * j + 1] += g.y * xh1;
+      db[2 * j] += g.x; db[2 * j + 1] += g.y;
+      s1[h] += d0 + d1;
+      s2[h] += d0 * xh0 + d1 * xh1;
+      acc[4 * j + 2 * h] = xh0; acc[4 * j + 2 * h + 1] = xh1;
+      dxh[4 * j + 2 * h] = d0; dxh[4 * j + 2 * h + 1] = d1;
+    }
+  }
+
+#pragma unroll
+  for (int h = 0; h < 2; ++h) {
+#pragma unroll
+    for (int o = 1; o <= 2; o <<= 1) {
+      s1[h] += __shfl_xor_sync(0xffffffffu, s1[h], o);
+      s2[h] += __shfl_xor_sync(0xffffffffu, s2[h], o);
+    }
+    st_async2(mapa(smem_addr(&red[rank][tr[h]]), q4), s1[h], s2[h], mapa(smem_addr(&red_bar[0]), q4));
+  }
+  mbar_wait(smem_addr(&red_bar[0]), 0);
+#pragma unroll
+  for (int h = 0; h < 2; ++h) {
+    const float2 a = red[0][tr[h]], b = red[1][tr[h]], c = red[2][tr[h]], d = red[3][tr[h]];
+    s1[h] = (((a.x + b.x) + c.x) + d.x) * (1.f / (CLUSTER * BN));
+    s2[h] = (((a.y + b.y) + c.y) + d.y) * (1.f / (CLUSTER * BN));
+  }
+
+#pragma unroll
+  for (int j = 0; j < BN / 8; ++j) {
+#pragma unroll
+    for (int h = 0; h < 2; ++h) {
+      const uint32_t o = frag_off(tr[h], j, q4);
+      const float dy0 = rstd[h] * (dxh[4 * j + 2 * h] - s1[h] - acc[4 * j + 2 * h] * s2[h]);
+      const float dy1 = rstd[h] * (dxh[4 * j + 2 * h + 1] - s1[h] - acc[4 * j + 2 * h + 1] * s2[h]);
+      const uint32_t mk = keep[h] >> (2 * j);
+      *reinterpret_cast<__nv_bfloat162*>(rt + o) = __floats2bfloat162_rn(dy0, dy1);
+      *reinterpret_cast<__nv_bfloat162*>(zt + o) =
+          __floats2bfloat162_rn((mk & 1) ? dy0 * keep_scale : 0.f, (mk & 2) ? dy1 * keep_scale : 0.f);
+    }
+  }
+  fence_proxy_async();
+  named_bar(2 + wg, 128);
+  if ((threadIdx.x & 127) == 0 && row0 < p.M) {
+    tma_store_2d(&tmDZ, smem_addr(zt + wg * 8192), n0, row0);
+    tma_store_2d(&tmDR, smem_addr(rt + wg * 8192), n0, row0);
+    asm volatile("cp.async.bulk.commit_group;" ::: "memory");
+  }
+
+#pragma unroll
+  for (int i = 0; i < BN / 4; ++i) {
+#pragma unroll
+    for (int o = 4; o < 32; o <<= 1) {
+      dg[i] += __shfl_xor_sync(0xffffffffu, dg[i], o);
+      db[i] += __shfl_xor_sync(0xffffffffu, db[i], o);
+    }
+  }
+  if (lane < 4) {
+#pragma unroll
+    for (int j = 0; j < BN / 8; ++j) {
+      *reinterpret_cast<float2*>(&colred[0][warp][8 * j + 2 * q4]) = make_float2(dg[2 * j], dg[2 * j + 1]);
+      *reinterpret_cast<float2*>(&colred[1][warp][8 * j + 2 * q4]) = make_float2(db[2 * j], db[2 * j + 1]);
+    }
+  }
+  named_bar(1, C::N_CONSUMER);
+  if (threadIdx.x < 2 * BN / 4) {
+    const int which = threadIdx.x / (BN / 4), c = (threadIdx.x % (BN / 4)) * 4;
+    float4 s = make_float4(0.f, 0.f, 0.f, 0.f);
+#pragma unroll
+    for (int w = 0; w < WG * 4; ++w) {
+      const float4 v = *reinterpret_cast<const float4*>(&colred[which][w][c]);
+      s.x += v.x; s.y += v.y; s.z += v.z; s.w += v.w;
+    }
+    atomicAdd(reinterpret_cast<float4*>((which ? p.d_beta : p.d_gamma) + n0 + c), s);
+  }
+  if ((threadIdx.x & 127) == 0) tma_store_commit_wait_read();
+}
+
+bool wide_tiles(long rows) { return (rows + 127) / 128 * CLUSTER >= fira_num_sms(); }
+
+template <typename Kern>
+int set_smem(Kern kernel, uint32_t smem, const char* who) {
+  cudaError_t e = cudaFuncSetAttribute(kernel, cudaFuncAttributeMaxDynamicSharedMemorySize, (int)smem);
+  if (e != cudaSuccess) { fira_set_error(FIRA_ERR_CUDA, "%s attr: %s", who, cudaGetErrorString(e)); return FIRA_ERR_CUDA; }
+  return FIRA_OK;
+}
+
+template <int WG>
+int gemm_ln_fwd_launch(const CUtensorMap& tx, const CUtensorMap& tw, const CUtensorMap& tr, const CUtensorMap& tz,
+                       const CUtensorMap& toa, const CUtensorMap& tob, const FwdParams& p, cudaStream_t st) {
+  using C = Cfg<WG>;
+  constexpr uint32_t smem = C::smem(2);
+  if (int rc = set_smem(gemm_ln_fwd_kernel<WG>, smem, "gemm_ln_fwd")) return rc;
+  launch_k_cluster(gemm_ln_fwd_kernel<WG>, dim3(CLUSTER, (p.M + C::BM - 1) / C::BM), dim3(C::THREADS), smem, st, CLUSTER,
+                   tx, tw, tr, tz, toa, tob, p);
+  return FIRA_OK;
+}
+
+template <int WG>
+int gemm_dx_ln_bwd_launch(const CUtensorMap* maps, const BwdParams& p, cudaStream_t st) {
+  using C = Cfg<WG>;
+  constexpr uint32_t smem = C::smem(3);
+  if (int rc = set_smem(gemm_dx_ln_bwd_kernel<WG>, smem, "gemm_dx_ln_bwd")) return rc;
+  launch_k_cluster(gemm_dx_ln_bwd_kernel<WG>, dim3(CLUSTER, (p.M + C::BM - 1) / C::BM), dim3(C::THREADS), smem, st, CLUSTER,
+                   maps[0], maps[1], maps[2], maps[3], maps[4], maps[5], maps[6], p);
+  return FIRA_OK;
 }
 
 }
@@ -202,21 +490,55 @@
   FIRA_CHECK_ARG(p_drop >= 0.f && p_drop < 1.f, FIRA_ERR_ARG, "gemm_ln_fwd: p_drop %f", p_drop);
   if (split > rows || outB == nullptr) split = rows;
   FIRA_CHECK_ARG(split >= 0, FIRA_ERR_ARG, "gemm_ln_fwd: split %ld", split);
-  const int M = (int)rows;
+  const int M = (int)rows, D = CLUSTER * BN;
+  const bool wide = wide_tiles(rows);
+  const int BM = wide ? 128 : 64;
   CUtensorMap tx, tw, tr, tz, toa, tob;
   int rc_;
   if ((rc_ = make_map_bf16(&tx, x, M, K, ldx, BK, BM, "gemm_ln_fwd"))) return rc_;
-  if ((rc_ = make_map_bf16(&tw, w, BN, K, K, BK, BN, "gemm_ln_fwd"))) return rc_;
-  if ((rc_ = make_map_bf16(&tr, resid, M, BN, BN, 64, BM, "gemm_ln_fwd"))) return rc_;
-  if ((rc_ = make_map_bf16(&tz, z, M, BN, BN, 64, 64, "gemm_ln_fwd"))) return rc_;
+  if ((rc_ = make_map_bf16(&tw, w, D, K, K, BK, BN, "gemm_ln_fwd"))) return rc_;
+  if ((rc_ = make_map_bf16(&tr, resid, M, D, D, BN, BM, "gemm_ln_fwd"))) return rc_;
+  if ((rc_ = make_map_bf16(&tz, z, M, D, D, BN, 64, "gemm_ln_fwd"))) return rc_;
   const bool has_a = split > 0, has_b = split < rows;
-  if ((rc_ = make_map_bf16(&toa, outA, has_a ? split : 1, BN, BN, 64, 64, "gemm_ln_fwd"))) return rc_;
+  if ((rc_ = make_map_bf16(&toa, outA, has_a ? split : 1, D, D, BN, 64, "gemm_ln_fwd"))) return rc_;
   tob = toa;
-  if (has_b && (rc_ = make_map_bf16(&tob, outB, rows, BN, BN, 64, 32, "gemm_ln_fwd"))) return rc_;
-  LnParams p{M, K, has_a ? split : 0, bias, rs, rc, gamma, beta, mean, rstd, p_drop, seed, seed_ctr, stream_id, has_b ? 1 : 0};
-  cudaError_t e = cudaFuncSetAttribute(gemm_ln_kernel, cudaFuncAttributeMaxDynamicSharedMemorySize, (int)SMEM_BYTES);
-  if (e != cudaSuccess) { fira_set_error(FIRA_ERR_CUDA, "gemm_ln attr: %s", cudaGetErrorString(e)); return FIRA_ERR_CUDA; }
-  launch_k(gemm_ln_kernel, dim3((M + BM - 1) / BM), dim3(THREADS), SMEM_BYTES, (cudaStream_t)stream, tx, tw, tr, tz, toa, tob, p);
+  if (has_b && (rc_ = make_map_bf16(&tob, outB, rows, D, D, BN, 32, "gemm_ln_fwd"))) return rc_;
+  FwdParams p{M, K, has_a ? split : 0, bias, rs, rc, gamma, beta, mean, rstd, p_drop, seed, seed_ctr, stream_id, has_b ? 1 : 0};
+  cudaStream_t st = (cudaStream_t)stream;
+  rc_ = wide ? gemm_ln_fwd_launch<2>(tx, tw, tr, tz, toa, tob, p, st) : gemm_ln_fwd_launch<1>(tx, tw, tr, tz, toa, tob, p, st);
+  if (rc_) return rc_;
   FIRA_CHECK_LAUNCH("fira_gemm_ln_fwd");
   return FIRA_OK;
 }
+
+extern "C" int fira_gemm_dx_ln_bwd(const void* dy, long lddy, const void* w, int K, const void* addend, const void* z,
+                                   const void* resid, const float* mean, const float* rstd, const float* gamma, void* d_z,
+                                   void* d_resid, float* d_gamma, float* d_beta, long rows, float p_drop, uint64_t seed,
+                                   const uint64_t* seed_ctr, uint32_t stream_id, void* stream) {
+  FIRA_CHECK_ARG(dy && w && addend && z && resid && mean && rstd && gamma && d_z && d_resid && d_gamma && d_beta, FIRA_ERR_ARG,
+                 "gemm_dx_ln_bwd: null argument");
+  FIRA_CHECK_ARG(rows > 0 && rows < (1L << 31) && K > 0 && K % 8 == 0, FIRA_ERR_SHAPE, "gemm_dx_ln_bwd: rows %ld K %d", rows, K);
+  FIRA_CHECK_ARG(lddy % 8 == 0, FIRA_ERR_ALIGN, "gemm_dx_ln_bwd: lddy must be a multiple of 8");
+  FIRA_CHECK_ARG(fira_aligned16(dy) && fira_aligned16(w) && fira_aligned16(addend) && fira_aligned16(z) && fira_aligned16(resid) &&
+                     fira_aligned16(d_z) && fira_aligned16(d_resid) && fira_aligned16(d_gamma) && fira_aligned16(d_beta),
+                 FIRA_ERR_ALIGN, "gemm_dx_ln_bwd: 16-B alignment");
+  FIRA_CHECK_ARG(p_drop >= 0.f && p_drop < 1.f, FIRA_ERR_ARG, "gemm_dx_ln_bwd: p_drop %f", p_drop);
+  const int M = (int)rows, D = CLUSTER * BN;
+  const bool wide = wide_tiles(rows);
+  const int BM = wide ? 128 : 64;
+  CUtensorMap maps[7];
+  int rc_;
+  if ((rc_ = make_map_bf16(&maps[0], dy, M, K, lddy, BK, BM, "gemm_dx_ln_bwd"))) return rc_;
+  if ((rc_ = make_map_bf16(&maps[1], w, K, D, D, BN, BK, "gemm_dx_ln_bwd"))) return rc_;
+  const void* in[3] = {z, resid, addend};
+  for (int t = 0; t < 3; ++t)
+    if ((rc_ = make_map_bf16(&maps[2 + t], in[t], M, D, D, BN, BM, "gemm_dx_ln_bwd"))) return rc_;
+  if ((rc_ = make_map_bf16(&maps[5], d_z, M, D, D, BN, 64, "gemm_dx_ln_bwd"))) return rc_;
+  if ((rc_ = make_map_bf16(&maps[6], d_resid, M, D, D, BN, 64, "gemm_dx_ln_bwd"))) return rc_;
+  BwdParams p{M, K, mean, rstd, gamma, d_gamma, d_beta, p_drop, seed, seed_ctr, stream_id};
+  cudaStream_t st = (cudaStream_t)stream;
+  rc_ = wide ? gemm_dx_ln_bwd_launch<2>(maps, p, st) : gemm_dx_ln_bwd_launch<1>(maps, p, st);
+  if (rc_) return rc_;
+  FIRA_CHECK_LAUNCH("fira_gemm_dx_ln_bwd");
+  return FIRA_OK;
+}
diff --git a/fira_icse_b200/ops.py b/fira_icse_b200/ops.py
--- a/fira_icse_b200/ops.py
+++ b/fira_icse_b200/ops.py
@@ -192,7 +192,7 @@
 
     def linear_ln(self, x, W, b, resid, gamma, beta, outA, outB, split, rows, p, seed, sid, rs=None, rc=None):
         N, K = W.shape
-        if self.bf16 and N == D and FUSE_GEMM_LN:
+        if self.bf16 and N == D and FUSE_GEMM_LN and rows <= _ln_fused_rows():
             z = torch.empty((rows, D), dtype=torch.bfloat16, device=x.device)
             stats = torch.empty((2, rows), dtype=torch.float32, device=x.device)
             call("fira_gemm_ln_fwd", _ptr(x), K, _ptr(self.w(W)), _ptr(b), _ptr(rs), _ptr(rc), _ptr(resid), _ptr(gamma),
@@ -219,6 +219,19 @@
              _ptr(self.seed_ctr), sid, self.code, _stream())
         return dz, d_resid, dgb[0], dgb[1]
 
+    def linear_dx_ln_bwd(self, dy, ld_dy, W, M, addend, z, resid, stats, gamma, p, seed, sid, beta=None):
+        N, K = W.shape
+        if not (self.bf16 and K == D and FUSE_GEMM_LN):
+            self.linear_dx(dy, ld_dy, W, M, out=addend, accumulate=True)
+            return self.ln_bwd(addend, addend, M, z, resid, stats, gamma, M, p, seed, sid, beta=beta)
+        dz, d_resid = torch.empty_like(z), torch.empty_like(z)
+        dgb = _gdest((gamma, beta), (2, D), zero=True) if beta is not None else \
+            torch.zeros((2, D), dtype=torch.float32, device=z.device)
+        call("fira_gemm_dx_ln_bwd", _ptr(dy), ld_dy, _ptr(self.w(W)), N, _ptr(addend), _ptr(z), _ptr(resid), _ptr(stats),
+             _ptr(stats, M), _ptr(gamma), _ptr(dz), _ptr(d_resid), _ptr(dgb), _ptr(dgb, D), M, float(p), seed,
+             _ptr(self.seed_ctr), sid, _stream())
+        return dz, d_resid, dgb[0], dgb[1]
+
 
 _F32 = Prec(False)
 
@@ -233,7 +246,11 @@
 
 _SIDE_STREAMS = {}
 N_SIDE = max(1, int(os.environ.get("FIRA_SIDE_STREAMS", "8")))
-FUSE_GEMM_LN = os.environ.get("FIRA_GEMM_LN", "0") != "0"
+FUSE_GEMM_LN = True
+
+
+def _ln_fused_rows():
+    return _num_sms() // 4 * 128
 FUSE_DX_RELU = os.environ.get("FIRA_DX_RELU", "1") != "0" and os.environ.get("FIRA_GEMM_TMA_STORE", "1") != "0"
 MERGE_SPLITS = max(1, int(os.environ.get("FIRA_MERGE_SPLITS", "4")))
 _TURN = [0]
@@ -606,13 +623,16 @@
         grads = [None] * len(lp)
         F = 4 * D
         fork = Fork(dev)
+        ffn_ln = None
         for i in reversed(range(L)):
             (sWq, sbq, sWk, sbk, sWv, sbv, sWo, sbo, slw, slb,
              cWq, cbq, cWk, cbk, cWv, cbv, cWo, cbo, clw, clb,
              fW1, fb1, fW2, fb2, flw, flb) = lp[i * 26:(i + 1) * 26]
             X, Wqkv, QKV, ctx1, st1, Z1, ls1, X1, Q, ctx2, st2, Z2, ls2, X2, Hh, Z3, ls3 = ctx.saved[i]
             sid = cfg["stream_base"] + 64 + i * 8
-            dZ3, dX2, d_flw, d_flb = pr.ln_bwd(dX, dX, Mt, Z3, X2, ls3, flw, Mt, p, seed, sid + 2, beta=flb)
+            if ffn_ln is None:
+                ffn_ln = pr.ln_bwd(dX, dX, Mt, Z3, X2, ls3, flw, Mt, p, seed, sid + 2, beta=flb)
+            dZ3, dX2, d_flw, d_flb = ffn_ln
             with fork(dZ3, Hh):
                 d_fb2 = _gdest(fb2, (D,), zero=True)
                 d_fW2 = pr.linear_dw(dZ3, D, Hh, F, Mt, D, F, out=_gdest(fW2, (D, F)), dbias=d_fb2)
@@ -620,8 +640,7 @@
             with fork(dHh, X2):
                 d_fb1 = _gdest(fb1, (F,), zero=True)
                 d_fW1 = pr.linear_dw(dHh, F, X2, D, Mt, F, D, out=_gdest(fW1, (F, D)), dbias=d_fb1)
-            pr.linear_dx(dHh, F, fW1, Mt, out=dX2, accumulate=True)
-            dZ2, dX1, d_clw, d_clb = pr.ln_bwd(dX2, dX2, Mt, Z2, X1, ls2, clw, Mt, p, seed, sid + 1, beta=clb)
+            dZ2, dX1, d_clw, d_clb = pr.linear_dx_ln_bwd(dHh, F, fW1, Mt, dX2, Z2, X1, ls2, clw, p, seed, sid + 1, beta=clb)
             with fork(dZ2, ctx2):
                 d_cbo = _gdest(cbo, (D,), zero=True)
                 d_cWo = pr.linear_dw(dZ2, D, ctx2, D, Mt, D, D, out=_gdest(cWo, (D, D)), dbias=d_cbo)
@@ -638,8 +657,7 @@
             with fork(dQ, X1):
                 d_cbq = _gdest(cbq, (D,), zero=True)
                 d_cWq = pr.linear_dw(dQ, D, X1, D, Mt, D, D, out=_gdest(cWq, (D, D)), dbias=d_cbq)
-            pr.linear_dx(dQ, D, cWq, Mt, out=dX1, accumulate=True)
-            dZ1, dX0, d_slw, d_slb = pr.ln_bwd(dX1, dX1, Mt, Z1, X, ls1, slw, Mt, p, seed, sid + 0, beta=slb)
+            dZ1, dX0, d_slw, d_slb = pr.linear_dx_ln_bwd(dQ, D, cWq, Mt, dX1, Z1, X, ls1, slw, p, seed, sid + 0, beta=slb)
             with fork(dZ1, ctx1):
                 d_sbo = _gdest(sbo, (D,), zero=True)
                 d_sWo = pr.linear_dw(dZ1, D, ctx1, D, Mt, D, D, out=_gdest(sWo, (D, D)), dbias=d_sbo)
@@ -651,7 +669,13 @@
             with fork(dQKV, X):
                 d_bqkv = _gdest((sbq, sbk, sbv), (3 * D,), zero=True)
                 d_Wqkv = pr.linear_dw(dQKV, 3 * D, X, D, Mt, 3 * D, D, out=_gdest((sWq, sWk, sWv), (3 * D, D)), dbias=d_bqkv)
-            pr.linear_dx(dQKV, 3 * D, Wqkv, Mt, out=dX0, accumulate=True)
+            if i > 0:
+                X2p, Z3p, ls3p = ctx.saved[i - 1][13], ctx.saved[i - 1][15], ctx.saved[i - 1][16]
+                flwp, flbp = lp[(i - 1) * 26 + 24], lp[(i - 1) * 26 + 25]
+                ffn_ln = pr.linear_dx_ln_bwd(dQKV, 3 * D, Wqkv, Mt, dX0, Z3p, X2p, ls3p, flwp, p, seed,
+                                             cfg["stream_base"] + 64 + (i - 1) * 8 + 2, beta=flbp)
+            else:
+                pr.linear_dx(dQKV, 3 * D, Wqkv, Mt, out=dX0, accumulate=True)
             grads[i * 26:(i + 1) * 26] = [
                 d_Wqkv[:D], d_bqkv[:D], d_Wqkv[D:2 * D], d_bqkv[D:2 * D], d_Wqkv[2 * D:], d_bqkv[2 * D:],
                 d_sWo, d_sbo, d_slw, d_slb,
diff --git a/include/fira_b200.h b/include/fira_b200.h
--- a/include/fira_b200.h
+++ b/include/fira_b200.h
@@ -35,6 +35,11 @@
                      const void* resid, const float* gamma, const float* beta, void* z, void* outA, void* outB, long split,
                      float* mean, float* rstd, long rows, int K, float p_drop, uint64_t seed, const uint64_t* seed_ctr,
                      uint32_t stream_id, void* stream);
+
+int fira_gemm_dx_ln_bwd(const void* dy, long lddy, const void* w, int K, const void* addend, const void* z,
+                        const void* resid, const float* mean, const float* rstd, const float* gamma, void* d_z,
+                        void* d_resid, float* d_gamma, float* d_beta, long rows, float p_drop, uint64_t seed,
+                        const uint64_t* seed_ctr, uint32_t stream_id, void* stream);
 
 int fira_gemm_bf16_tc_dx_relu(const void* dy, long lddy, const void* W, long ldw, void* dx, long lddx, const void* h,
                               int M, int N, int K, void* stream);
```

Result: faster. 18320, median of 6 (+1.3%).
